# Alanlee0323/ISWM

Hardware: AMD Instinct MI355X
Metric: training images/sec (513x513) DeepLabV3+-ResNet101 (higher is better)
Workload: dtype f32; 1 GPU; deeplabv3plus_resnet101 output_stride=16, 513x513 synthetic tiles, 16 images/GPU (BASELINE.json configs[2]: global batch 128 over 8 GPUs), weighted CE [1,3], SGD-nesterov + cosine LR; fp32 tensors, conv products via six bf16 MFMAs on an exact 3-way operand split (bf16x6, fp32-level error); conv_math=bf16x6, global_batch=16, parallelism=dp1

## Files before the change

### include/iswm_hip.h

```cpp
#ifndef ISWM_HIP_H
#define ISWM_HIP_H

#include <stddef.h>
#include <stdint.h>

#ifdef __cplusplus
extern "C" {
#endif

typedef void* iswm_stream_t;

const char* iswm_last_error(void);
int iswm_version(void);

typedef struct {
    int N, H, W, Cin;
    int Ho, Wo, Cout;
    int KH, KW, stride, pad, dil;
    int ldx;
    int ldy;
} iswm_conv_desc;

int iswm_set_conv_math(int mode);
int iswm_get_conv_math(void);
int iswm_conv2d_kernel_name(const iswm_conv_desc* d, int kind, char* buf, int buflen);
int iswm_conv2d_stat_tile_rows(const iswm_conv_desc* d);
int iswm_conv2d_stat_tiles(const iswm_conv_desc* d);
int iswm_conv2d_fwd(const iswm_conv_desc* d, const float* x, const float* w, const float* bias,
                    float* y, float* stat_partials, iswm_stream_t stream);
int iswm_conv2d_dgrad(const iswm_conv_desc* d, const float* dy, const float* w, float* dx,
                      int accumulate, iswm_stream_t stream);
int iswm_transpose_weights(const iswm_conv_desc* d, const float* w, float* wt, iswm_stream_t stream);
int iswm_conv2d_dgrad_wants_wt(const iswm_conv_desc* d);
int iswm_conv2d_dgrad_wt(const iswm_conv_desc* d, const float* dy, const float* wt, float* dx, int accumulate,
                         iswm_stream_t stream);
size_t iswm_conv2d_packed_weight_bytes(const iswm_conv_desc* d, int kind);
int iswm_conv2d_pack_weights(const iswm_conv_desc* d, int kind, const float* w, void* packed, iswm_stream_t stream);
typedef struct iswm_pack_job {
    const float* w;
    void* packed;
    int Cout, taps, Cin, kind;
    int first_block, reserved;
} iswm_pack_job;
size_t iswm_packed_weight_bytes(int Cout, int taps, int Cin, int kind);
int iswm_pack_job_blocks(int Cout, int taps, int Cin, int kind);
int iswm_pack_weights_batch(const iswm_pack_job* jobs_dev, int njobs, int total_blocks, iswm_stream_t stream);
int iswm_conv2d_fwd_packed_stat_layout(const iswm_conv_desc* d, int* tiles, int* tile_rows);
int iswm_conv2d_fwd_packed(const iswm_conv_desc* d, const float* x, const void* wpk, const float* bias,
                           float* y, float* stat_partials, iswm_stream_t stream);
int iswm_conv2d_dgrad_packed(const iswm_conv_desc* d, const float* dy, const void* wpk, float* dx, int accumulate,
                             iswm_stream_t stream);
int iswm_split_planes(const float* x, int64_t M, int C, int ldx, void* planes, int ldp, int64_t plane_stride,
                      iswm_stream_t stream);
int iswm_join_planes(const void* planes, int ldp, int64_t plane_stride, int64_t M, int C, float* x, int ldx,
                     iswm_stream_t stream);
int iswm_bn_apply_pl(const float* y, int64_t M, int C, int ldy, const float* scale, const float* shift, const float* mean,
                     const void* residual, int ldr, int64_t res_ps, int relu, void* out, int ldo, int64_t out_ps,
                     iswm_stream_t stream);
int iswm_bn_backward_pl(const float* dout, int ldd, const void* out, int ldo, int64_t out_ps, const float* y, int ldy,
                        int64_t M, int C, const float* mean, const float* invstd, const float* gamma,
                        const float* mask_scale, const float* mask_shift, int relu, int training, float* dgamma,
                        float* dbeta, void* dy, int lddy, int64_t dy_ps, float* dres, int lddres, void* workspace,
                        size_t workspace_bytes, iswm_stream_t stream);
int iswm_maxpool3x3s2_fwd_pl(const float* x, int N, int H, int W, int C, void* y, int64_t y_ps, uint8_t* idx, int Ho,
                             int Wo, iswm_stream_t stream);
int iswm_gap_fwd_pl(const void* x, int64_t x_ps, int N, int HW, int C, int ldx, float* y, iswm_stream_t stream);
int iswm_bcast_fwd_pl(const float* v, int N, int HW, int C, void* y, int ldy, int64_t y_ps, iswm_stream_t stream);
int iswm_bilinear_fwd_pl(const float* x, int N, int Hi, int Wi, int C, int ldx, void* y, int64_t y_ps, int Ho, int Wo,
                         int ldy, iswm_stream_t stream);
size_t iswm_conv2d_pl2_weight_bytes(const iswm_conv_desc* d, int kind);
int iswm_conv2d_pl2_pack_weights(const iswm_conv_desc* d, int kind, const float* w, void* packed, iswm_stream_t stream);
int iswm_conv2d_pl2_tile_rows(const iswm_conv_desc* d, int kind);
int iswm_conv2d_fwd_pl2(const iswm_conv_desc* d, const void* xp, int64_t plane_stride, const void* wpk,
                        const float* bias, float* y, float* stat_partials, iswm_stream_t stream);
int iswm_conv2d_dgrad_pl2(const iswm_conv_desc* d, const void* dyp, int64_t plane_stride, const void* wpk,
                          float* dx, int accumulate, iswm_stream_t stream);
int iswm_conv2d_dgrad_pl2_stat_tiles(const iswm_conv_desc* d);
int iswm_conv2d_dgrad_pl2_bn(const iswm_conv_desc* d, const void* dyp, int64_t plane_stride, const void* wpk, float* dx,
                             int accumulate, const float* y, int ldy, const float* mean, const float* invstd,
                             const float* mask_scale, const float* mask_shift, int relu, const void* mask_hi,
                             int ld_mask, double* partials, int tiles, iswm_stream_t stream);
int iswm_bn_backward_stats_pl(const float* dout, int ldd, const void* out, int ldo, int64_t out_ps, const float* y, int ldy,
                              int64_t M, int C, const float* mean, const float* invstd, const float* gamma,
                              const float* mask_scale, const float* mask_shift, int relu, int training, float* dgamma,
                              float* dbeta, void* dy, int lddy, int64_t dy_ps, float* dres, int lddres,
                              const double* partials, int tiles, void* workspace, size_t workspace_bytes,
                              iswm_stream_t stream);
size_t iswm_aspp_plan_bytes(const iswm_conv_desc* d, int nbranch, const int* ksize, const int* dil, int kind);
int iswm_aspp_plan(const iswm_conv_desc* d, int nbranch, const int* ksize, const int* dil, int kind, void* host_plan,
                   int grid_hint);
int iswm_aspp_fwd(const iswm_conv_desc* d, int nbranch, const int* ksize, const int* dil, const void* plan_dev, const void* xp,
                  int64_t x_ps, const void* const* wpk, float* const* y, float* const* stats, iswm_stream_t stream);
int iswm_aspp_bwd(const iswm_conv_desc* d, int nbranch, const int* ksize, const int* dil, const void* plan_dev, const void* dyp,
                  int64_t dy_ps, int ld_dy, const void* const* wpk, float* dx, int accumulate, const void* xp, int64_t x_ps,
                  float* const* dw, float* workspace, size_t workspace_bytes, iswm_stream_t stream);
int iswm_conv2d_wgrad_planes_ok(const iswm_conv_desc* d);
size_t iswm_conv2d_wgrad_planes_workspace(const iswm_conv_desc* d);
int iswm_conv2d_wgrad_planes(const iswm_conv_desc* d, const void* xp, int64_t x_ps, const void* dyp, int64_t dy_ps, float* dw,
                             float* workspace, size_t workspace_bytes, iswm_stream_t stream);
int iswm_dwconv2d_fwd(const iswm_conv_desc* d, const float* x, const float* w, int Cw, const float* bias, float* y,
                      iswm_stream_t stream);
int iswm_dwconv2d_dgrad(const iswm_conv_desc* d, const float* dy, const float* w, int Cw, float* dx, int accumulate,
                        iswm_stream_t stream);
size_t iswm_dwconv2d_wgrad_workspace(const iswm_conv_desc* d);
int iswm_dwconv2d_wgrad(const iswm_conv_desc* d, const float* x, const float* dy, int Cw, float* dw, void* workspace,
                        size_t workspace_bytes, iswm_stream_t stream);
int iswm_dwconv3x3_stat_tile_rows(const iswm_conv_desc* d);
int iswm_dwconv3x3_stat_tiles(const iswm_conv_desc* d);
int iswm_dwconv3x3_fwd_stats(const iswm_conv_desc* d, const float* x, const float* w, int Cw, float* y,
                             float* stat_partials, iswm_stream_t stream);
size_t iswm_dwconv3x3_bwd_workspace(const iswm_conv_desc* d);
int iswm_dwconv3x3_bwd(const iswm_conv_desc* d, const float* x, const float* dy, const float* w, int Cw, float* dx,
                       int lddx, int accumulate, float* dw, void* workspace, size_t workspace_bytes, iswm_stream_t stream);
size_t iswm_conv2d_wgrad_workspace(const iswm_conv_desc* d);
int iswm_conv2d_wgrad(const iswm_conv_desc* d, const float* x, const float* dy, float* dw,
                      float* workspace, size_t workspace_bytes, iswm_stream_t stream);

int iswm_colstat_tiles(int64_t M);
int64_t iswm_colstat_tile_rows(int64_t M);
int iswm_colstat(const float* x, int64_t M, int C, int ld, float* partials, iswm_stream_t stream);
int iswm_bn_finalize(const float* partials, int tiles, int C, int64_t count, int64_t tile_rows,
                     const float* gamma, const float* beta, float* running_mean, float* running_var, float momentum,
                     float eps, float* scale, float* shift, float* save_mean, float* save_invstd,
                     iswm_stream_t stream);
int iswm_colstat_res(const float* x, int64_t M, int C, int ld, float* partials, iswm_stream_t stream);
int iswm_bn_finalize_res(const float* partials, int tiles, int C, int64_t count, int64_t tile_rows,
                         const float* gamma, const float* beta, float* running_mean, float* running_var, float momentum,
                         float eps, float* scale, float* shift, float* save_mean, float* save_invstd,
                         iswm_stream_t stream);
int iswm_bn_eval_coeffs(int C, const float* gamma, const float* beta, const float* running_mean,
                        const float* running_var, float eps, float* scale, float* shift,
                        float* save_mean, float* save_invstd, iswm_stream_t stream);
int iswm_bn_apply(const float* y, int64_t M, int C, int ldy, const float* scale, const float* shift,
                  const float* mean, const float* residual, int ldr, int relu, float* out, int ldo,
                  iswm_stream_t stream);
size_t iswm_bn_bwd_workspace(int64_t M, int C);
int iswm_bn_backward(const float* dout, int ldd, const float* out, int ldo, const float* y, int ldy,
                     int64_t M, int C, const float* mean, const float* invstd, const float* gamma,
                     const float* mask_scale, const float* mask_shift,
                     int relu, int training, float* dgamma, float* dbeta, float* dy, int lddy,
                     float* dres, int lddres, void* workspace, size_t workspace_bytes,
                     iswm_stream_t stream);
int iswm_colsum_finalize(const float* partials, int tiles, int C, float* out, float* scratch,
                         iswm_stream_t stream);

int iswm_maxpool3x3s2_fwd(const float* x, int N, int H, int W, int C, float* y, uint8_t* idx, int Ho,
                          int Wo, iswm_stream_t stream);
int iswm_maxpool3x3s2_bwd(const float* dy, const uint8_t* idx, int N, int H, int W, int C, int Ho,
                          int Wo, float* dx, iswm_stream_t stream);
int iswm_gap_fwd(const float* x, int N, int HW, int C, int ldx, float* y, iswm_stream_t stream);
int iswm_gap_bwd(const float* dy, int N, int HW, int C, float* dx, int lddx, int accumulate,
                 iswm_stream_t stream);
int iswm_bcast_fwd(const float* v, int N, int HW, int C, float* y, int ldy, iswm_stream_t stream);
int iswm_bcast_bwd(const float* dy, int lddy, int N, int HW, int C, float* dv, iswm_stream_t stream);

int iswm_bilinear_fwd(const float* x, int N, int Hi, int Wi, int C, int ldx, float* y, int Ho, int Wo,
                      int ldy, iswm_stream_t stream);
int iswm_bilinear_bwd(const float* dy, int N, int Hi, int Wi, int C, int lddy, int Ho, int Wo, float* dx,
                      int lddx, iswm_stream_t stream);
int iswm_bilinear_nhwc_to_nchw_fwd(const float* x, int N, int Hi, int Wi, int C, int ldx, float* y,
                                   int Ho, int Wo, iswm_stream_t stream);
int iswm_bilinear_nhwc_to_nchw_bwd(const float* dy, int N, int Hi, int Wi, int C, int lddx, int Ho,
                                   int Wo, float* dx, iswm_stream_t stream);

int iswm_nchw_to_nhwc(const float* x, int N, int C, int HW, float* y, int Cp, iswm_stream_t stream);
int iswm_nhwc_to_nchw(const float* x, int N, int C, int HW, int ldx, float* y, iswm_stream_t stream);
int iswm_copy_channels(const float* src, int lds, float* dst, int ldd, int64_t M, int C,
                       iswm_stream_t stream);
int iswm_add_inplace(float* dst, const float* src, int64_t n, iswm_stream_t stream);
int iswm_scale_inplace(float* x, int64_t n, const float* scalar_dev, float host_mul, iswm_stream_t stream);
int iswm_bn_apply_classify(const float* y, int64_t M, int C, int ldy, const float* scale, const float* shift, const float* mean,
                           const float* wc4, const float* bias4, float* logits, int ldl, iswm_stream_t stream);
size_t iswm_bn_classify_bwd_workspace(int64_t M, int C);
int iswm_bn_backward_classify(const float* dlogit, int ldl, const float* wc4, const float* y, int ldy, int64_t M, int C,
                              const float* mean, const float* invstd, const float* gamma, const float* mask_scale,
                              const float* mask_shift, int training, float* dgamma, float* dbeta, float* dwc4, void* dy, int lddy,
                              int64_t dy_ps, void* workspace, size_t workspace_bytes, iswm_stream_t stream);
int iswm_pad_weights(const float* w, int cout, int cin, int kh, int kw, const int64_t* strides, int cout_p, int cin_p, float* out_ohwi,
                     iswm_stream_t stream);
int iswm_unpad_weights(const float* dw_ohwi, int cout_p, int cin_p, int cout, int cin, int kh, int kw, float* grad,
                       const int64_t* strides, iswm_stream_t stream);
int iswm_fill_zero(void* p, size_t bytes, iswm_stream_t stream);
int iswm_zero_cols(void* y, int64_t M, int64_t ld_bytes, int byte0, int byte1, int64_t plane_bytes, int nplanes, iswm_stream_t stream);
int iswm_dropout_fwd(const float* x, float* y, uint8_t* mask, int64_t n, float p, uint64_t seed,
                     uint64_t offset, iswm_stream_t stream);
int iswm_dropout_bwd(const float* dy, const uint8_t* mask, float* dx, int64_t n, float p,
                     iswm_stream_t stream);

int iswm_loss_blocks(int64_t npix);
int iswm_loss_fwd(const float* logits, const void* labels, int label_bytes, int B, int C, int64_t HW,
                  const float* class_weight, int ignore_index, float alpha, float gamma, int mode,
                  float* grad_unnorm, float* partials, iswm_stream_t stream);
int iswm_loss_finalize(const float* partials, int blocks, int mode, int64_t npix, float* sums,
                       float* loss, iswm_stream_t stream);
int iswm_loss_bwd_scale(float* grad, int64_t n, const float* sums, const float* upstream, int mode,
                        int64_t npix, iswm_stream_t stream);
int iswm_overlap_loss_fwd(const float* logits, const void* labels, int label_bytes, int B, int C, int64_t HW,
                          const float* class_weight, int ignore_index, float* partials, double* sums,
                          iswm_stream_t stream);
int iswm_overlap_loss_coeffs(const double* sums, int C, double ce_weight, double overlap_weight, double alpha,
                             double beta, double gamma, double smooth, int classes, float* loss, float* coef,
                             iswm_stream_t stream);
int iswm_overlap_loss_bwd(const float* logits, const void* labels, int label_bytes, int B, int C, int64_t HW,
                          const float* class_weight, int ignore_index, const float* coef, const float* upstream,
                          float* grad, iswm_stream_t stream);
int iswm_argmax_nchw(const float* logits, int B, int C, int64_t HW, int64_t* out, iswm_stream_t stream);

int iswm_confusion_matrix(const void* labels, int label_dtype, const void* preds, int pred_dtype, int64_t npix,
                          int n_classes, int64_t* hist, iswm_stream_t stream);
int iswm_confusion_matrix_logits(const void* labels, int label_dtype, const float* logits, int B, int C, int64_t HW,
                                 int n_classes, int64_t* hist, iswm_stream_t stream);

int iswm_mask_morph(const void* src, int src_dtype, int N, int H, int W, int radius, int dilate, uint8_t* dst,
                    iswm_stream_t stream);
int iswm_ccl(const uint8_t* mask, int N, int H, int W, int32_t* labels, int32_t* areas, iswm_stream_t stream);
size_t iswm_mask_preprocess_workspace(int N, int H, int W);
int iswm_mask_preprocess(const void* src, int src_dtype, int N, int H, int W, uint8_t* out, double* weight,
                         int64_t* area, void* workspace, size_t workspace_bytes, iswm_stream_t stream);
int iswm_mask_fronts(const uint8_t* mask, const double* weight, int N, int H, int W, int32_t* fronts, int64_t* stats,
// ... 148 lines not shown
```

### iswm_amd/_lib.py

```python
import ctypes
import os
from ctypes import POINTER, Structure, c_char_p, c_double, c_float, c_int, c_int64, c_size_t, c_uint64, c_void_p

HERE = os.path.dirname(os.path.abspath(__file__))
LIB_PATH = os.path.join(HERE, "libiswm_hip.so")


class ConvDesc(Structure):
    _fields_ = [(n, c_int) for n in ("N", "H", "W", "Cin", "Ho", "Wo", "Cout", "KH", "KW", "stride", "pad",
                                     "dil", "ldx", "ldy")]


class QConvDesc(Structure):
    _fields_ = [(n, c_int) for n in ("N", "H", "W", "Cin", "Ho", "Wo", "Cout", "KH", "KW", "stride", "pad",
                                     "dil", "ldx", "ldy", "ldr", "relu", "lo", "out_f32", "cstore")]


class ScenePlan(Structure):
    _fields_ = [(n, c_int) for n in ("H", "W", "th", "tw", "sy", "sx", "nty", "ntx", "ramp")]

    @property
    def ntiles(self):
        return self.nty * self.ntx

    def origins_y(self):
        return [min(k * self.sy, self.H - self.th) for k in range(self.nty)]

    def origins_x(self):
        return [min(k * self.sx, self.W - self.tw) for k in range(self.ntx)]

    def astuple(self):
        return tuple(getattr(self, n) for n, _ in self._fields_)


class PredictView(Structure):
    _fields_ = [("yl", c_void_p), ("Hi", c_int), ("Wi", c_int), ("flip", c_int)]


P = c_void_p
_SIGS = {
    "iswm_last_error": (c_char_p, []),
    "iswm_version": (c_int, []),
    "iswm_set_conv_math": (c_int, [c_int]),
    "iswm_get_conv_math": (c_int, []),
    "iswm_conv2d_kernel_name": (c_int, [POINTER(ConvDesc), c_int, c_char_p, c_int]),
    "iswm_conv2d_stat_tile_rows": (c_int, [POINTER(ConvDesc)]),
    "iswm_conv2d_stat_tiles": (c_int, [POINTER(ConvDesc)]),
    "iswm_conv2d_fwd": (c_int, [POINTER(ConvDesc), P, P, P, P, P, P]),
    "iswm_conv2d_dgrad": (c_int, [POINTER(ConvDesc), P, P, P, c_int, P]),
    "iswm_transpose_weights": (c_int, [POINTER(ConvDesc), P, P, P]),
    "iswm_conv2d_dgrad_wants_wt": (c_int, [POINTER(ConvDesc)]),
    "iswm_conv2d_dgrad_wt": (c_int, [POINTER(ConvDesc), P, P, P, c_int, P]),
    "iswm_conv2d_packed_weight_bytes": (c_size_t, [POINTER(ConvDesc), c_int]),
    "iswm_conv2d_pack_weights": (c_int, [POINTER(ConvDesc), c_int, P, P, P]),
    "iswm_packed_weight_bytes": (c_size_t, [c_int, c_int, c_int, c_int]),
    "iswm_pack_job_blocks": (c_int, [c_int, c_int, c_int, c_int]),
    "iswm_pack_weights_batch": (c_int, [P, c_int, c_int, P]),
    "iswm_conv2d_fwd_packed_stat_layout": (c_int, [POINTER(ConvDesc), POINTER(c_int), POINTER(c_int)]),
    "iswm_conv2d_fwd_packed": (c_int, [POINTER(ConvDesc), P, P, P, P, P, P]),
    "iswm_conv2d_dgrad_packed": (c_int, [POINTER(ConvDesc), P, P, P, c_int, P]),
    "iswm_split_planes": (c_int, [P, c_int64, c_int, c_int, P, c_int, c_int64, P]),
    "iswm_join_planes": (c_int, [P, c_int, c_int64, c_int64, c_int, P, c_int, P]),
    "iswm_bn_apply_pl": (c_int, [P, c_int64, c_int, c_int, P, P, P, P, c_int, c_int64, c_int, P, c_int, c_int64, P]),
    "iswm_bn_backward_pl": (c_int, [P, c_int, P, c_int, c_int64, P, c_int, c_int64, c_int, P, P, P, P, P, c_int, c_int, P, P, P,
                                    c_int, c_int64, P, c_int, P, c_size_t, P]),
    "iswm_maxpool3x3s2_fwd_pl": (c_int, [P, c_int, c_int, c_int, c_int, P, c_int64, P, c_int, c_int, P]),
    "iswm_gap_fwd_pl": (c_int, [P, c_int64, c_int, c_int, c_int, c_int, P, P]),
    "iswm_bcast_fwd_pl": (c_int, [P, c_int, c_int, c_int, P, c_int, c_int64, P]),
    "iswm_bilinear_fwd_pl": (c_int, [P, c_int, c_int, c_int, c_int, c_int, P, c_int64, c_int, c_int, c_int, P]),
    "iswm_conv2d_pl2_weight_bytes": (c_size_t, [POINTER(ConvDesc), c_int]),
    "iswm_conv2d_pl2_pack_weights": (c_int, [POINTER(ConvDesc), c_int, P, P, P]),
    "iswm_conv2d_pl2_tile_rows": (c_int, [POINTER(ConvDesc), c_int]),
    "iswm_conv2d_fwd_pl2": (c_int, [POINTER(ConvDesc), P, c_int64, P, P, P, P, P]),
    "iswm_conv2d_dgrad_pl2": (c_int, [POINTER(ConvDesc), P, c_int64, P, P, c_int, P]),
    "iswm_conv2d_dgrad_pl2_stat_tiles": (c_int, [POINTER(ConvDesc)]),
    "iswm_conv2d_dgrad_pl2_bn": (c_int, [POINTER(ConvDesc), P, c_int64, P, P, c_int, P, c_int, P, P, P, P, c_int, P, c_int, P,
                                         c_int, P]),
    "iswm_bn_backward_stats_pl": (c_int, [P, c_int, P, c_int, c_int64, P, c_int, c_int64, c_int, P, P, P, P, P, c_int, c_int, P, P,
                                          P, c_int, c_int64, P, c_int, P, c_int, P, c_size_t, P]),
    "iswm_aspp_plan_bytes": (c_size_t, [POINTER(ConvDesc), c_int, POINTER(c_int), POINTER(c_int), c_int]),
    "iswm_aspp_plan": (c_int, [POINTER(ConvDesc), c_int, POINTER(c_int), POINTER(c_int), c_int, P, c_int]),
    "iswm_aspp_fwd": (c_int, [POINTER(ConvDesc), c_int, POINTER(c_int), POINTER(c_int), P, P, c_int64, POINTER(c_void_p),
                              POINTER(c_void_p), POINTER(c_void_p), P]),
    "iswm_aspp_bwd": (c_int, [POINTER(ConvDesc), c_int, POINTER(c_int), POINTER(c_int), P, P, c_int64, c_int, POINTER(c_void_p), P,
                              c_int, P, c_int64, POINTER(c_void_p), P, c_size_t, P]),
    "iswm_conv2d_wgrad_planes_ok": (c_int, [POINTER(ConvDesc)]),
    "iswm_conv2d_wgrad_planes_workspace": (c_size_t, [POINTER(ConvDesc)]),
    "iswm_conv2d_wgrad_planes": (c_int, [POINTER(ConvDesc), P, c_int64, P, c_int64, P, P, c_size_t, P]),
    "iswm_conv2d_wgrad_workspace": (c_size_t, [POINTER(ConvDesc)]),
    "iswm_dwconv2d_fwd": (c_int, [POINTER(ConvDesc), P, P, c_int, P, P, P]),
    "iswm_dwconv2d_dgrad": (c_int, [POINTER(ConvDesc), P, P, c_int, P, c_int, P]),
    "iswm_dwconv2d_wgrad_workspace": (c_size_t, [POINTER(ConvDesc)]),
    "iswm_dwconv2d_wgrad": (c_int, [POINTER(ConvDesc), P, P, c_int, P, P, c_size_t, P]),
    "iswm_dwconv3x3_stat_tile_rows": (c_int, [POINTER(ConvDesc)]),
    "iswm_dwconv3x3_stat_tiles": (c_int, [POINTER(ConvDesc)]),
    "iswm_dwconv3x3_fwd_stats": (c_int, [POINTER(ConvDesc), P, P, c_int, P, P, P]),
    "iswm_dwconv3x3_bwd_workspace": (c_size_t, [POINTER(ConvDesc)]),
    "iswm_dwconv3x3_bwd": (c_int, [POINTER(ConvDesc), P, P, P, c_int, P, c_int, c_int, P, P, c_size_t, P]),
    "iswm_conv2d_wgrad": (c_int, [POINTER(ConvDesc), P, P, P, P, c_size_t, P]),
    "iswm_colstat_tiles": (c_int, [c_int64]),
    "iswm_colstat_tile_rows": (c_int64, [c_int64]),
    "iswm_colstat": (c_int, [P, c_int64, c_int, c_int, P, P]),
    "iswm_bn_finalize": (c_int, [P, c_int, c_int, c_int64, c_int64, P, P, P, P, c_float, c_float, P, P, P, P, P]),
    "iswm_colstat_res": (c_int, [P, c_int64, c_int, c_int, P, P]),
    "iswm_bn_finalize_res": (c_int, [P, c_int, c_int, c_int64, c_int64, P, P, P, P, c_float, c_float, P, P, P, P, P]),
    "iswm_bn_eval_coeffs": (c_int, [c_int, P, P, P, P, c_float, P, P, P, P, P]),
    "iswm_bn_apply": (c_int, [P, c_int64, c_int, c_int, P, P, P, P, c_int, c_int, P, c_int, P]),
    "iswm_bn_bwd_workspace": (c_size_t, [c_int64, c_int]),
    "iswm_bn_backward": (c_int, [P, c_int, P, c_int, P, c_int, c_int64, c_int, P, P, P, P, P, c_int, c_int, P, P, P, c_int,
                                 P, c_int, P, c_size_t, P]),
    "iswm_colsum_finalize": (c_int, [P, c_int, c_int, P, P, P]),
    "iswm_maxpool3x3s2_fwd": (c_int, [P, c_int, c_int, c_int, c_int, P, P, c_int, c_int, P]),
    "iswm_maxpool3x3s2_bwd": (c_int, [P, P, c_int, c_int, c_int, c_int, c_int, c_int, P, P]),
    "iswm_gap_fwd": (c_int, [P, c_int, c_int, c_int, c_int, P, P]),
    "iswm_gap_bwd": (c_int, [P, c_int, c_int, c_int, P, c_int, c_int, P]),
    "iswm_bcast_fwd": (c_int, [P, c_int, c_int, c_int, P, c_int, P]),
    "iswm_bcast_bwd": (c_int, [P, c_int, c_int, c_int, c_int, P, P]),
    "iswm_bilinear_fwd": (c_int, [P, c_int, c_int, c_int, c_int, c_int, P, c_int, c_int, c_int, P]),
    "iswm_bilinear_bwd": (c_int, [P, c_int, c_int, c_int, c_int, c_int, c_int, c_int, P, c_int, P]),
    "iswm_bilinear_nhwc_to_nchw_fwd": (c_int, [P, c_int, c_int, c_int, c_int, c_int, P, c_int, c_int, P]),
    "iswm_bilinear_nhwc_to_nchw_bwd": (c_int, [P, c_int, c_int, c_int, c_int, c_int, c_int, c_int, P, P]),
    "iswm_nchw_to_nhwc": (c_int, [P, c_int, c_int, c_int, P, c_int, P]),
    "iswm_nhwc_to_nchw": (c_int, [P, c_int, c_int, c_int, c_int, P, P]),
    "iswm_copy_channels": (c_int, [P, c_int, P, c_int, c_int64, c_int, P]),
    "iswm_add_inplace": (c_int, [P, P, c_int64, P]),
    "iswm_scale_inplace": (c_int, [P, c_int64, P, c_float, P]),
    "iswm_bn_apply_classify": (c_int, [P, c_int64, c_int, c_int, P, P, P, P, P, P, c_int, P]),
    "iswm_bn_classify_bwd_workspace": (c_size_t, [c_int64, c_int]),
    "iswm_bn_backward_classify": (c_int, [P, c_int, P, P, c_int, c_int64, c_int, P, P, P, P, P, c_int, P, P, P, P, c_int, c_int64,
                                          P, c_size_t, P]),
    "iswm_pad_weights": (c_int, [P, c_int, c_int, c_int, c_int, P, c_int, c_int, P, P]),
    "iswm_unpad_weights": (c_int, [P, c_int, c_int, c_int, c_int, c_int, c_int, P, P, P]),
    "iswm_fill_zero": (c_int, [P, c_size_t, P]),
    "iswm_zero_cols": (c_int, [P, c_int64, c_int64, c_int, c_int, c_int64, c_int, P]),
    "iswm_dropout_fwd": (c_int, [P, P, P, c_int64, c_float, c_uint64, c_uint64, P]),
    "iswm_dropout_bwd": (c_int, [P, P, P, c_int64, c_float, P]),
    "iswm_loss_blocks": (c_int, [c_int64]),
    "iswm_loss_fwd": (c_int, [P, P, c_int, c_int, c_int, c_int64, P, c_int, c_float, c_float, c_int, P, P, P]),
    "iswm_loss_finalize": (c_int, [P, c_int, c_int, c_int64, P, P, P]),
    "iswm_loss_bwd_scale": (c_int, [P, c_int64, P, P, c_int, c_int64, P]),
    "iswm_overlap_loss_fwd": (c_int, [P, P, c_int, c_int, c_int, c_int64, P, c_int, P, P, P]),
    "iswm_overlap_loss_coeffs": (c_int, [P, c_int, c_double, c_double, c_double, c_double, c_double, c_double, c_int, P, P, P]),
    "iswm_overlap_loss_bwd": (c_int, [P, P, c_int, c_int, c_int, c_int64, P, c_int, P, P, P, P]),
    "iswm_argmax_nchw": (c_int, [P, c_int, c_int, c_int64, P, P]),
    "iswm_augment_batch": (c_int, [P, P, P, P, c_int, c_int, c_int, POINTER(c_float), POINTER(c_float), P, P, P]),
    "iswm_aug_rotate": (c_int, [P, P, P, P, c_int, c_int64, P, c_size_t, P, c_size_t, P]),
    "iswm_augment_batch_ex_workspace": (c_size_t, [c_int, c_int, c_int]),
    "iswm_augment_batch_ex": (c_int, [P, P, P, P, P, P, P, c_int, c_int, c_int, POINTER(c_float), POINTER(c_float), c_int, P,
                                      P, P, c_size_t, P]),
    "iswm_label_prepare_workspace": (c_size_t, [c_int64]),
    "iswm_label_prepare": (c_int, [P, c_int64, P, P, c_size_t, P]),
    "iswm_label_count_workspace": (c_size_t, [c_int64]),
    "iswm_label_count": (c_int, [P, c_int64, c_int, P, P, c_size_t, P]),
    "iswm_aug_tables_workspace": (c_size_t, [P, c_int]),
    "iswm_aug_tables": (c_int, [P, c_int, c_int, P, c_size_t, P]),
    "iswm_gather_normalize": (c_int, [P, P, P, c_int, c_int, c_int, POINTER(c_float), POINTER(c_float), P, P, P]),
    "iswm_confusion_matrix": (c_int, [P, c_int, P, c_int, c_int64, c_int, P, P]),
    "iswm_confusion_matrix_logits": (c_int, [P, c_int, P, c_int, c_int, c_int64, c_int, P, P]),
    "iswm_mask_morph": (c_int, [P, c_int, c_int, c_int, c_int, c_int, c_int, P, P]),
    "iswm_ccl": (c_int, [P, c_int, c_int, c_int, P, P, P]),
    "iswm_mask_preprocess_workspace": (c_size_t, [c_int, c_int, c_int]),
    "iswm_mask_preprocess": (c_int, [P, c_int, c_int, c_int, c_int, P, P, P, P, c_size_t, P]),
    "iswm_mask_fronts": (c_int, [P, P, c_int, c_int, c_int, P, P, P]),
    "iswm_front_error": (c_int, [P, P, c_int, c_int, c_double, P, P]),
    "iswm_mask_pair_scores": (c_int, [P, P, P, P, P, c_int, c_int, c_int, P, P, P]),
    "iswm_region_workspace": (c_size_t, [c_int, c_int, c_int]),
    "iswm_region_score": (c_int, [P, c_int, P, c_int, c_int, c_int, c_int, P, P, P, c_size_t, P]),
    "iswm_predict_normalize": (c_int, [P, c_int, c_int, c_int, POINTER(c_float), POINTER(c_float), P, P]),
    "iswm_predict_maps_workspace": (c_size_t, [c_int, c_int, c_int]),
    "iswm_predict_maps": (c_int, [P, c_int, c_int, c_int, c_int, c_int, c_int, c_int, c_int, c_float, c_int, c_int, P, P,
                                  P, P, P, P, c_size_t, P]),
    "iswm_scene_plan_make": (c_int, [c_int, c_int, c_int, c_int, POINTER(ScenePlan)]),
    "iswm_scene_tiles_normalize": (c_int, [P, POINTER(ScenePlan), c_int, c_int, POINTER(c_float), POINTER(c_float), P, P]),
    "iswm_scene_maps_workspace": (c_size_t, [c_int, c_int]),
    "iswm_scene_maps": (c_int, [P, POINTER(ScenePlan), c_int, c_int, c_int, c_int, c_int, c_float, c_int, c_int, P, P, P, P,
                                P, P, c_size_t, P]),
    "iswm_predict_view_normalize": (c_int, [P, c_int, c_int, c_int, c_int, c_int, c_int, POINTER(c_float), POINTER(c_float),
                                            P, P]),
    "iswm_predict_views_maps_workspace": (c_size_t, [c_int, c_int, c_int]),
    "iswm_predict_views_maps": (c_int, [POINTER(PredictView), c_int, c_int, c_int, c_int, c_int, c_int, c_int, c_float,
                                        c_int, c_int, P, P, P, P, P, P, c_size_t, P]),
    "iswm_val_panels": (c_int, [P, P, P, c_int, c_int, c_int, c_int, c_int, c_int, c_int, c_int, POINTER(c_float),
                                POINTER(c_float), P, P, P, P, P, P, P, P, P, P]),
    "iswm_qconv_weight_bytes": (c_size_t, [POINTER(QConvDesc)]),
    "iswm_qconv_fwd": (c_int, [POINTER(QConvDesc), P, P, P, P, P, c_double, c_double, P, P]),
    "iswm_absmax_workspace": (c_size_t, [c_int64, c_int]),
    "iswm_absmax": (c_int, [P, c_int64, c_int64, c_int, c_int, P, c_size_t, P, P]),
    "iswm_quantize_i8": (c_int, [P, c_int64, c_int64, c_int, c_int, c_double, c_int, P, c_int, P]),
    "iswm_qgap": (c_int, [P, c_int, c_int, c_int, c_int, c_double, c_double, P, c_int, P]),
    "iswm_qbcast": (c_int, [P, c_int, c_int, c_int, c_int, P, c_int, P]),
    "iswm_qbilinear": (c_int, [P, c_int, c_int, c_int, c_int, c_int, c_double, c_int, c_int, c_double, P, c_int, P]),
    "iswm_sgd_step": (c_int, [P, P, P, c_int64, P, c_float, c_float, c_int, P]),
    "iswm_adam_step": (c_int, [P, P, P, P, c_int64, P, c_float, c_float, c_float, c_float, c_int, P]),
    "iswm_grad_sqnorm_slots": (c_int, []),
    "iswm_grad_sqnorm": (c_int, [P, c_int64, P, c_int, P]),
    "iswm_clip_finalize": (c_int, [P, c_float, P, P]),
    "iswm_sgd_step_ex": (c_int, [P, P, P, c_int64, P, c_float, c_float, c_int, P, P, P]),
    "iswm_adam_step_ex": (c_int, [P, P, P, P, c_int64, P, c_float, c_float, c_float, c_float, c_int, P, P, P]),
    "iswm_swap_f32": (c_int, [P, P, c_int64, P]),
}

EXPORTS = tuple(_SIGS)
_lib = None


class IswmError(RuntimeError):
    pass


def load():
    global _lib
    if _lib is not None:
        return _lib
    if not os.path.exists(LIB_PATH):
        raise ImportError(
            "libiswm_hip.so is not built (%s). Run `python -m iswm_amd.build` (hipcc, gfx950). "
            "iswm_amd has no CPU or torch-op fallback." % LIB_PATH)
    import torch
    lib = ctypes.CDLL(LIB_PATH)
    for name, (res, args) in _SIGS.items():
# ... 14 lines not shown
```

### iswm_amd/csrc/bn.hip

```cpp
#include <stdlib.h>

#include "rowmap.h"

namespace iswm {

template <bool RES>
__global__ __launch_bounds__(256) void k_colstat(const float* __restrict__ x, int64_t M, int C4, int ld,
                                                 int CQ, int RL, int tiles, int C, int64_t R,
                                                 float* __restrict__ partials) {
    __shared__ float red[256 * 4];
    __shared__ float mean_s[256 * 4];
    RowThread rt = row_thread(C4, CQ, RL);
    const int t = threadIdx.x;
    const int64_t r_begin = (int64_t)blockIdx.x * R;
    const int64_t r_end = min(M, r_begin + R);
    const float cnt = (float)(r_end - r_begin);
    const float* p = x + rt.c4 * 4;
    float4 s = make_float4(0, 0, 0, 0);
    if (rt.active)
        for (int64_t r = r_begin + rt.rl; r < r_end; r += RL) {
            float4 v = ld4(p + r * ld);
            s.x += v.x; s.y += v.y; s.z += v.z; s.w += v.w;
        }
    st4(&red[t * 4], s);
    __syncthreads();
    if (rt.active && rt.rl == 0) {
        for (int k = 1; k < RL; ++k) {
            float4 a = ld4(&red[(t + k * CQ) * 4]);
            s.x += a.x; s.y += a.y; s.z += a.z; s.w += a.w;
        }
        st4(&partials[(size_t)blockIdx.x * C + rt.c4 * 4], s);
        st4(&mean_s[t * 4], make_float4(s.x / cnt, s.y / cnt, s.z / cnt, s.w / cnt));
    }
    __syncthreads();
    float4 q = make_float4(0, 0, 0, 0), rs = q;
    if (rt.active) {
        const float4 mu = ld4(&mean_s[(t - rt.rl * CQ) * 4]);
        for (int64_t r = r_begin + rt.rl; r < r_end; r += RL) {
            float4 v = ld4(p + r * ld);
            float dx = v.x - mu.x, dy = v.y - mu.y, dz = v.z - mu.z, dw = v.w - mu.w;
            q.x += dx * dx; q.y += dy * dy; q.z += dz * dz; q.w += dw * dw;
            if (RES) { rs.x += dx; rs.y += dy; rs.z += dz; rs.w += dw; }
        }
    }
    st4(&red[t * 4], q);
    __syncthreads();
    if (rt.active && rt.rl == 0) {
        for (int k = 1; k < RL; ++k) {
            float4 a = ld4(&red[(t + k * CQ) * 4]);
            q.x += a.x; q.y += a.y; q.z += a.z; q.w += a.w;
        }
        st4(&partials[(size_t)(tiles + blockIdx.x) * C + rt.c4 * 4], q);
    }
    if (RES) {
        __syncthreads();
        st4(&red[t * 4], rs);
        __syncthreads();
        if (rt.active && rt.rl == 0) {
            for (int k = 1; k < RL; ++k) {
                float4 a = ld4(&red[(t + k * CQ) * 4]);
                rs.x += a.x; rs.y += a.y; rs.z += a.z; rs.w += a.w;
            }
            st4(&partials[(size_t)(2 * tiles + blockIdx.x) * C + rt.c4 * 4], rs);
        }
    }
}

template <int CPB>
__global__ __launch_bounds__(256) void k_bn_finalize(const float* __restrict__ partials, int tiles, int C,
                                                     double count, double R, const float* __restrict__ gamma,
                                                     const float* __restrict__ beta, float* running_mean,
                                                     float* running_var, float momentum, float eps,
                                                     float* scale, float* shift, float* save_mean,
                                                     float* save_invstd) {
    constexpr int TL = 256 / CPB;
    __shared__ double red[TL][CPB + 1];
    __shared__ double mean_s[CPB];
    const int cl = threadIdx.x % CPB, tl = threadIdx.x / CPB;
    const int c = blockIdx.x * CPB + cl;
    constexpr int KEEP = 8;
    float sv[KEEP], qv[KEEP];
    double s = 0.0;
    if (c < C) {
#pragma unroll
        for (int i = 0; i < KEEP; ++i) {
            const int k = tl + i * TL;
            sv[i] = k < tiles ? partials[(size_t)k * C + c] : 0.f;
            qv[i] = k < tiles ? partials[(size_t)(tiles + k) * C + c] : 0.f;
        }
#pragma unroll
        for (int i = 0; i < KEEP; ++i) s += (double)sv[i];
        for (int k = tl + KEEP * TL; k < tiles; k += TL) s += (double)partials[(size_t)k * C + c];
    }
    red[tl][cl] = s;
    __syncthreads();
    if (tl == 0) {
        for (int k = 1; k < TL; ++k) s += red[k][cl];
        mean_s[cl] = s / count;
    }
    __syncthreads();
    const double mean = mean_s[cl];
    double m2 = 0.0;
    if (c < C) {
        auto term = [&](int k, float sk, float qk) -> double {
            const double nt = R > 0.0 ? fmin(R, count - (double)k * R) : (double)partials[(size_t)2 * tiles * C + k];
            const double d = (double)sk / nt - mean;
            return (double)qk + nt * d * d;
        };
#pragma unroll
        for (int i = 0; i < KEEP; ++i) {
            const int k = tl + i * TL;
            if (k < tiles) m2 += term(k, sv[i], qv[i]);
        }
        for (int k = tl + KEEP * TL; k < tiles; k += TL) m2 += term(k, partials[(size_t)k * C + c], partials[(size_t)(tiles + k) * C + c]);
    }
    __syncthreads();
    red[tl][cl] = m2;
    __syncthreads();
    if (tl == 0 && c < C) {
        for (int k = 1; k < TL; ++k) m2 += red[k][cl];
        double var = m2 / count;
        if (var < 0.0) var = 0.0;
        float invstd = (float)(1.0 / sqrt(var + (double)eps));
        float g = gamma ? gamma[c] : 1.f, b = beta ? beta[c] : 0.f;
        float sc = g * invstd;
        scale[c] = sc;
        shift[c] = b;
        save_mean[c] = (float)mean;
        save_invstd[c] = invstd;
        if (running_mean) {
            double unbiased = count > 1.0 ? var * count / (count - 1.0) : var;
            running_mean[c] = (1.f - momentum) * running_mean[c] + momentum * (float)mean;
            running_var[c] = (1.f - momentum) * running_var[c] + momentum * (float)unbiased;
        }
    }
}

__global__ __launch_bounds__(256) void k_bn_finalize_res(const float* __restrict__ partials, int tiles, int C, double count,
                                                         double R, const float* __restrict__ gamma,
                                                         const float* __restrict__ beta, float* running_mean,
                                                         float* running_var, float momentum, float eps, float* scale,
                                                         float* shift, float* save_mean, float* save_invstd) {
    constexpr int CPB = 4, TL = 64;
    __shared__ double red[TL][CPB + 1];
    __shared__ double mean_s[CPB];
    const int cl = threadIdx.x % CPB, tl = threadIdx.x / CPB;
    const int c = blockIdx.x * CPB + cl;
    auto rows = [&](int k) -> double { return fmin(R, count - (double)k * R); };
    auto centre = [&](int k) -> double { return (double)(partials[(size_t)k * C + c] / (float)rows(k)); };
    double s = 0.0;
    if (c < C)
        for (int k = tl; k < tiles; k += TL) s += rows(k) * centre(k) + (double)partials[(size_t)(2 * tiles + k) * C + c];
    red[tl][cl] = s;
    __syncthreads();
    if (tl == 0) {
        for (int k = 1; k < TL; ++k) s += red[k][cl];
        mean_s[cl] = s / count;
    }
    __syncthreads();
    const double mean = mean_s[cl];
    double m2 = 0.0;
    if (c < C)
        for (int k = tl; k < tiles; k += TL) {
            const double d = centre(k) - mean;
            m2 += (double)partials[(size_t)(tiles + k) * C + c] + 2.0 * d * (double)partials[(size_t)(2 * tiles + k) * C + c] +
                  rows(k) * d * d;
        }
    __syncthreads();
    red[tl][cl] = m2;
    __syncthreads();
    if (tl == 0 && c < C) {
        for (int k = 1; k < TL; ++k) m2 += red[k][cl];
        double var = m2 / count;
        if (var < 0.0) var = 0.0;
        const float invstd = (float)(1.0 / sqrt(var + (double)eps));
        const float g = gamma ? gamma[c] : 1.f, b = beta ? beta[c] : 0.f;
        scale[c] = g * invstd;
        shift[c] = b;
        save_mean[c] = (float)mean;
        save_invstd[c] = invstd;
        if (running_mean) {
            const double unbiased = count > 1.0 ? var * count / (count - 1.0) : var;
            running_mean[c] = (1.f - momentum) * running_mean[c] + momentum * (float)mean;
            running_var[c] = (1.f - momentum) * running_var[c] + momentum * (float)unbiased;
        }
    }
}

__global__ void k_bn_eval_coeffs(int C, const float* gamma, const float* beta, const float* rm,
                                 const float* rv, float eps, float* scale, float* shift, float* save_mean,
                                 float* save_invstd) {
    int c = blockIdx.x * blockDim.x + threadIdx.x;
    if (c >= C) return;
    float invstd = 1.f / sqrtf(rv[c] + eps);
    float g = gamma ? gamma[c] : 1.f, b = beta ? beta[c] : 0.f;
    float sc = g * invstd;
    scale[c] = sc;
    shift[c] = b;
    save_mean[c] = rm[c];
    save_invstd[c] = invstd;
}

template <int RELU, bool RES>
__global__ __launch_bounds__(256) void k_bn_apply(const float* __restrict__ y, int64_t M, int C4, int ldy,
                                                  const float* __restrict__ scale,
                                                  const float* __restrict__ shift,
                                                  const float* __restrict__ mean,
                                                  const void* __restrict__ res, int ldr, int64_t rps,
                                                  void* __restrict__ out, int ldo, int64_t ops, int CQ, int RL) {
    RowThread rt = row_thread(C4, CQ, RL);
    if (!rt.active) return;
    const int c = rt.c4 * 4;
    const float4 sc = ld4(scale + c), sh = ld4(shift + c), mu = ld4(mean + c);
    for (int64_t r = rt.row0; r < M; r += rt.rstep) {
        float4 v = ld4(y + r * ldy + c);
        float4 o;
        o.x = (v.x - mu.x) * sc.x + sh.x; o.y = (v.y - mu.y) * sc.y + sh.y;
        o.z = (v.z - mu.z) * sc.z + sh.z; o.w = (v.w - mu.w) * sc.w + sh.w;
        if (RES) {
            float4 q = ld4x(res, r * ldr + c, rps);
            o.x += q.x; o.y += q.y; o.z += q.z; o.w += q.w;
        }
        if (RELU) {
            o.x = fmaxf(o.x, 0.f); o.y = fmaxf(o.y, 0.f); o.z = fmaxf(o.z, 0.f); o.w = fmaxf(o.w, 0.f);
        }
        if (RELU == 2) {
            o.x = fminf(o.x, 6.f); o.y = fminf(o.y, 6.f); o.z = fminf(o.z, 6.f); o.w = fminf(o.w, 6.f);
        }
        st4x(out, r * ldo + c, ops, o);
    }
}

template <int RELU, bool RES>
__global__ __launch_bounds__(256) void k_bn_apply8(const float* __restrict__ y, int64_t M, int C8, int ldy,
                                                   const float* __restrict__ scale, const float* __restrict__ shift,
                                                   const float* __restrict__ mean, const void* __restrict__ res, int ldr,
                                                   int64_t rps, void* __restrict__ out, int ldo, int64_t ops, int CQ, int RL) {
    RowThread rt = row_thread(C8, CQ, RL);
    if (!rt.active) return;
    const int c = rt.c4 * 8;
    const float4 sc0 = ld4(scale + c), sc1 = ld4(scale + c + 4), sh0 = ld4(shift + c), sh1 = ld4(shift + c + 4);
    const float4 mu0 = ld4(mean + c), mu1 = ld4(mean + c + 4);
    auto one = [&](int64_t r, const float4 v0, const float4 v1, const float4 q0, const float4 q1) {
        float4 o0, o1;
        o0.x = (v0.x - mu0.x) * sc0.x + sh0.x; o0.y = (v0.y - mu0.y) * sc0.y + sh0.y;
        o0.z = (v0.z - mu0.z) * sc0.z + sh0.z; o0.w = (v0.w - mu0.w) * sc0.w + sh0.w;
        o1.x = (v1.x - mu1.x) * sc1.x + sh1.x; o1.y = (v1.y - mu1.y) * sc1.y + sh1.y;
        o1.z = (v1.z - mu1.z) * sc1.z + sh1.z; o1.w = (v1.w - mu1.w) * sc1.w + sh1.w;
        if (RES) {
            o0.x += q0.x; o0.y += q0.y; o0.z += q0.z; o0.w += q0.w;
            o1.x += q1.x; o1.y += q1.y; o1.z += q1.z; o1.w += q1.w;
        }
        if (RELU) {
            o0.x = fmaxf(o0.x, 0.f); o0.y = fmaxf(o0.y, 0.f); o0.z = fmaxf(o0.z, 0.f); o0.w = fmaxf(o0.w, 0.f);
            o1.x = fmaxf(o1.x, 0.f); o1.y = fmaxf(o1.y, 0.f); o1.z = fmaxf(o1.z, 0.f); o1.w = fmaxf(o1.w, 0.f);
        }
        if (RELU == 2) {
            o0.x = fminf(o0.x, 6.f); o0.y = fminf(o0.y, 6.f); o0.z = fminf(o0.z, 6.f); o0.w = fminf(o0.w, 6.f);
            o1.x = fminf(o1.x, 6.f); o1.y = fminf(o1.y, 6.f); o1.z = fminf(o1.z, 6.f); o1.w = fminf(o1.w, 6.f);
        }
        st8x(out, r * ldo + c, ops, o0, o1);
    };
    int64_t r = rt.row0;
    const float4 z4 = make_float4(0.f, 0.f, 0.f, 0.f);
    for (; r + rt.rstep < M; r += 2 * rt.rstep) {
        const int64_t r2 = r + rt.rstep;
        const float4 a0 = ld4(y + r * ldy + c), a1 = ld4(y + r * ldy + c + 4);
        const float4 b0 = ld4(y + r2 * ldy + c), b1 = ld4(y + r2 * ldy + c + 4);
        float4 qa0 = z4, qa1 = z4, qb0 = z4, qb1 = z4;
        if (RES) {
            ld8x(res, r * ldr + c, rps, qa0, qa1);
            ld8x(res, r2 * ldr + c, rps, qb0, qb1);
        }
        one(r, a0, a1, qa0, qa1);
        one(r2, b0, b1, qb0, qb1);
    }
    if (r < M) {
        const float4 a0 = ld4(y + r * ldy + c), a1 = ld4(y + r * ldy + c + 4);
        float4 qa0 = z4, qa1 = z4;
        if (RES) ld8x(res, r * ldr + c, rps, qa0, qa1);
        one(r, a0, a1, qa0, qa1);
    }
}

template <int RELU, bool DBL>
__global__ __launch_bounds__(256) void k_bn_bwd_reduce(const float* __restrict__ dout, int ldd,
                                                       const void* __restrict__ out, int ldo, int64_t ops,
                                                       const float* __restrict__ y, int ldy, int64_t M,
                                                       int C4, int C, const float* __restrict__ mean,
                                                       const float* __restrict__ invstd,
                                                       const float* __restrict__ mscale,
                                                       const float* __restrict__ mshift, int CQ, int RL,
                                                       int tiles, double* __restrict__ partials) {
    __shared__ double red[2 * 256 * 4];
    RowThread rt = row_thread(C4, CQ, RL);
    double s[4] = {0, 0, 0, 0}, s2[4] = {0, 0, 0, 0};
    if (rt.active) {
        const int c = rt.c4 * 4;
        const float4 mu = ld4(mean + c), is = ld4(invstd + c);
        float4 msc = make_float4(0.f, 0.f, 0.f, 0.f), msh = msc;
        if (RELU == 2) {
            msc = ld4(mscale + c);
            msh = ld4(mshift + c);
        }
        for (int64_t r = rt.row0; r < M; r += 8 * rt.rstep) {
            float f[4] = {0.f, 0.f, 0.f, 0.f}, f2[4] = {0.f, 0.f, 0.f, 0.f};
#pragma unroll
            for (int u = 0; u < 8; ++u) {
                const int64_t rr = r + u * rt.rstep;
                if (rr < M) {
                    float4 g = ld4(dout + rr * ldd + c);
                    float4 v = ld4(y + rr * ldy + c);
                    if (RELU == 1) {
                        float4 o = ld4x_hi(out, rr * ldo + c, ops);
                        g.x = o.x > 0.f ? g.x : 0.f; g.y = o.y > 0.f ? g.y : 0.f;
                        g.z = o.z > 0.f ? g.z : 0.f; g.w = o.w > 0.f ? g.w : 0.f;
                    } else if (RELU == 3) {
                        float4 o = ld4x_hi(out, rr * ldo + c, ops);
                        g.x = (o.x > 0.f && o.x < 6.f) ? g.x : 0.f; g.y = (o.y > 0.f && o.y < 6.f) ? g.y : 0.f;
                        g.z = (o.z > 0.f && o.z < 6.f) ? g.z : 0.f; g.w = (o.w > 0.f && o.w < 6.f) ? g.w : 0.f;
                    } else if (RELU == 2) {
                        g.x = (v.x - mu.x) * msc.x + msh.x > 0.f ? g.x : 0.f;
                        g.y = (v.y - mu.y) * msc.y + msh.y > 0.f ? g.y : 0.f;
                        g.z = (v.z - mu.z) * msc.z + msh.z > 0.f ? g.z : 0.f;
                        g.w = (v.w - mu.w) * msc.w + msh.w > 0.f ? g.w : 0.f;
                    }
                    if (DBL) {
                        const double gd[4] = {g.x, g.y, g.z, g.w}, vd[4] = {v.x, v.y, v.z, v.w};
                        const double mud[4] = {mu.x, mu.y, mu.z, mu.w}, isd[4] = {is.x, is.y, is.z, is.w};
#pragma unroll
                        for (int k = 0; k < 4; ++k) {
                            s[k] += gd[k];
                            s2[k] += gd[k] * ((vd[k] - mud[k]) * isd[k]);
                        }
                    } else {
                        f[0] += g.x; f[1] += g.y; f[2] += g.z; f[3] += g.w;
                        f2[0] += g.x * ((v.x - mu.x) * is.x); f2[1] += g.y * ((v.y - mu.y) * is.y);
                        f2[2] += g.z * ((v.z - mu.z) * is.z); f2[3] += g.w * ((v.w - mu.w) * is.w);
                    }
                }
            }
#pragma unroll
            for (int k = 0; k < 4; ++k) {
                s[k] += (double)f[k];
                s2[k] += (double)f2[k];
            }
        }
    }
    const int t = threadIdx.x;
#pragma unroll
    for (int k = 0; k < 4; ++k) {
        red[t * 4 + k] = s[k];
        red[(256 + t) * 4 + k] = s2[k];
    }
    __syncthreads();
    if (rt.active && rt.rl == 0) {
        for (int j = 1; j < RL; ++j)
#pragma unroll
            for (int k = 0; k < 4; ++k) {
                s[k] += red[(t + j * CQ) * 4 + k];
                s2[k] += red[(256 + t + j * CQ) * 4 + k];
            }
#pragma unroll
        for (int k = 0; k < 4; ++k) {
            partials[(size_t)blockIdx.x * C + rt.c4 * 4 + k] = s[k];
            partials[(size_t)(tiles + blockIdx.x) * C + rt.c4 * 4 + k] = s2[k];
        }
    }
}

template <typename T, int CPB>
__global__ __launch_bounds__(256) void k_bn_bwd_finalize(const T* __restrict__ partials, int tiles, int C,
                                                         float* dgamma, float* dbeta, double* sums) {
    constexpr int TL = 256 / CPB;
    __shared__ double red[2][TL][CPB + 1];
    const int cl = threadIdx.x % CPB, tl = threadIdx.x / CPB;
    const int c = blockIdx.x * CPB + cl;
    double s = 0.0, s2 = 0.0;
    if (c < C) {
        int k = tl;
        for (; k + TL < tiles; k += 2 * TL) {
            const T a0 = partials[(size_t)k * C + c], a1 = partials[(size_t)(k + TL) * C + c];
            const T b0 = partials[(size_t)(tiles + k) * C + c], b1 = partials[(size_t)(tiles + k + TL) * C + c];
            s += (double)a0 + (double)a1;
            s2 += (double)b0 + (double)b1;
        }
        for (; k < tiles; k += TL) {
            s += (double)partials[(size_t)k * C + c];
            s2 += (double)partials[(size_t)(tiles + k) * C + c];
        }
    }
    red[0][tl][cl] = s;
    red[1][tl][cl] = s2;
    __syncthreads();
    if (tl == 0 && c < C) {
        for (int k = 1; k < TL; ++k) {
            s += red[0][k][cl];
            s2 += red[1][k][cl];
        }
        dbeta[c] = (float)s;
        dgamma[c] = (float)s2;
        if (sums) {
            sums[c] = s;
            sums[C + c] = s2;
        }
    }
}

template <int RELU, bool TRAIN, bool DRES>
__global__ __launch_bounds__(256) void k_bn_bwd_apply(const float* __restrict__ dout, int ldd,
                                                      const void* __restrict__ out, int ldo, int64_t ops,
                                                      const float* __restrict__ y, int ldy, int64_t M,
                                                      int C4, int C, const float* __restrict__ mean,
                                                      const float* __restrict__ invstd,
                                                      const float* __restrict__ gamma,
                                                      const float* __restrict__ mscale,
                                                      const float* __restrict__ mshift,
                                                      const double* __restrict__ sums, double inv_count,
                                                      void* __restrict__ dy, int lddy, int64_t dyps,
                                                      float* __restrict__ dres, int lddres, int CQ, int RL) {
    RowThread rt = row_thread(C4, CQ, RL);
    if (!rt.active) return;
    const int c = rt.c4 * 4;
    const float4 mu = ld4(mean + c), is = ld4(invstd + c);
    const float4 ga = gamma ? ld4(gamma + c) : make_float4(1.f, 1.f, 1.f, 1.f);
    const double mud[4] = {mu.x, mu.y, mu.z, mu.w}, isd[4] = {is.x, is.y, is.z, is.w};
    const double gi[4] = {(double)ga.x * is.x, (double)ga.y * is.y, (double)ga.z * is.z, (double)ga.w * is.w};
    float4 msc = make_float4(0.f, 0.f, 0.f, 0.f), msh = msc;
    if (RELU == 2) {
        msc = ld4(mscale + c);
        msh = ld4(mshift + c);
    }
    double k1[4] = {0, 0, 0, 0}, k2[4] = {0, 0, 0, 0};
    if (TRAIN) {
#pragma unroll
        for (int k = 0; k < 4; ++k) {
            k1[k] = sums[c + k] * inv_count;
            k2[k] = sums[C + c + k] * inv_count;
        }
    }
    for (int64_t r = rt.row0; r < M; r += rt.rstep) {
        float4 g = ld4(dout + r * ldd + c);
        float4 v = make_float4(0.f, 0.f, 0.f, 0.f);
        if (TRAIN || RELU == 2) v = ld4(y + r * ldy + c);
        if (RELU == 1) {
            float4 o = ld4x_hi(out, r * ldo + c, ops);
            g.x = o.x > 0.f ? g.x : 0.f; g.y = o.y > 0.f ? g.y : 0.f;
            g.z = o.z > 0.f ? g.z : 0.f; g.w = o.w > 0.f ? g.w : 0.f;
        } else if (RELU == 3) {
            float4 o = ld4x_hi(out, r * ldo + c, ops);
            g.x = (o.x > 0.f && o.x < 6.f) ? g.x : 0.f; g.y = (o.y > 0.f && o.y < 6.f) ? g.y : 0.f;
            g.z = (o.z > 0.f && o.z < 6.f) ? g.z : 0.f; g.w = (o.w > 0.f && o.w < 6.f) ? g.w : 0.f;
        } else if (RELU == 2) {
            g.x = (v.x - mu.x) * msc.x + msh.x > 0.f ? g.x : 0.f;
            g.y = (v.y - mu.y) * msc.y + msh.y > 0.f ? g.y : 0.f;
            g.z = (v.z - mu.z) * msc.z + msh.z > 0.f ? g.z : 0.f;
            g.w = (v.w - mu.w) * msc.w + msh.w > 0.f ? g.w : 0.f;
        }
        if (DRES) st4(dres + r * lddres + c, g);
        const double gd[4] = {g.x, g.y, g.z, g.w};
        float d[4];
        if (TRAIN) {
            const double vd[4] = {v.x, v.y, v.z, v.w};
#pragma unroll
            for (int k = 0; k < 4; ++k)
                d[k] = (float)(gi[k] * (gd[k] - k1[k] - (vd[k] - mud[k]) * isd[k] * k2[k]));
        } else {
#pragma unroll
            for (int k = 0; k < 4; ++k) d[k] = (float)(gi[k] * gd[k]);
        }
        st4x(dy, r * lddy + c, dyps, make_float4(d[0], d[1], d[2], d[3]));
    }
}

static int chk_rows(const char* what, int64_t M, int C, int ld) {
    ISWM_REQUIRE(M > 0 && C > 0 && C % 4 == 0 && ld % 4 == 0 && ld >= C, "%s: bad shape M=%lld C=%d ld=%d", what,
                 (long long)M, C, ld);
    return 0;
}

}

using namespace iswm;

extern "C" int iswm_colstat_tiles(int64_t M) {
    int64_t t = (M + 31) / 32;
    if (t > 1024) t = 1024;
    if (t < 1) t = 1;
    return (int)t;
}

extern "C" int64_t iswm_colstat_tile_rows(int64_t M) {
    const int64_t tiles = iswm_colstat_tiles(M);
    return (M + tiles - 1) / tiles;
}

extern "C" int iswm_colstat(const float* x, int64_t M, int C, int ld, float* partials, iswm_stream_t stream) {
    if (int e = chk_rows("colstat", M, C, ld)) return e;
    ISWM_REQUIRE(x && partials && aligned16(x) && aligned16(partials), "colstat: bad pointer");
    const int64_t R = iswm_colstat_tile_rows(M);
    const int tiles = (int)((M + R - 1) / R);
    RowPlan p = plan_rows(M, C, tiles);
    hipLaunchKernelGGL((k_colstat<false>), dim3(p.rowblocks, p.colblocks), dim3(256), 0, (hipStream_t)stream, x, M, p.C4,
                       ld, p.CQ, p.RL, tiles, C, R, partials);
    return check_launch("colstat");
}

extern "C" int iswm_colstat_res(const float* x, int64_t M, int C, int ld, float* partials, iswm_stream_t stream) {
    if (int e = chk_rows("colstat_res", M, C, ld)) return e;
    ISWM_REQUIRE(x && partials && aligned16(x) && aligned16(partials), "colstat_res: bad pointer");
    const int64_t R = iswm_colstat_tile_rows(M);
    const int tiles = (int)((M + R - 1) / R);
    RowPlan p = plan_rows(M, C, tiles);
    hipLaunchKernelGGL((k_colstat<true>), dim3(p.rowblocks, p.colblocks), dim3(256), 0, (hipStream_t)stream, x, M, p.C4,
                       ld, p.CQ, p.RL, tiles, C, R, partials);
    return check_launch("colstat_res");
}

extern "C" int iswm_bn_finalize(const float* partials, int tiles, int C, int64_t count, int64_t tile_rows,
                                const float* gamma, const float* beta, float* running_mean, float* running_var, float momentum,
                                float eps, float* scale, float* shift, float* save_mean, float* save_invstd,
                                iswm_stream_t stream) {
    ISWM_REQUIRE(partials && scale && shift && save_mean && save_invstd && tiles > 0 && C > 0 && count > 0 &&
                     tile_rows >= 0 && (tile_rows == 0 || (int64_t)tiles == (count + tile_rows - 1) / tile_rows),
                 "bn_finalize: bad argument (tiles %d, count %lld, tile_rows %lld)", tiles, (long long)count,
                 (long long)tile_rows);
    if (tiles > 512)
        hipLaunchKernelGGL((k_bn_finalize<1>), dim3(C), dim3(256), 0, (hipStream_t)stream, partials, tiles, C,
                           (double)count, (double)tile_rows, gamma, beta, running_mean, running_var, momentum, eps,
                           scale, shift, save_mean, save_invstd);
    else if (tiles > 32)
        hipLaunchKernelGGL((k_bn_finalize<4>), dim3((C + 3) / 4), dim3(256), 0, (hipStream_t)stream, partials, tiles, C,
                           (double)count, (double)tile_rows, gamma, beta, running_mean, running_var, momentum, eps,
                           scale, shift, save_mean, save_invstd);
    else
        hipLaunchKernelGGL((k_bn_finalize<16>), dim3((C + 15) / 16), dim3(256), 0, (hipStream_t)stream, partials, tiles,
                           C, (double)count, (double)tile_rows, gamma, beta, running_mean, running_var, momentum, eps,
                           scale, shift, save_mean, save_invstd);
    return check_launch("bn_finalize");
}

extern "C" int iswm_bn_finalize_res(const float* partials, int tiles, int C, int64_t count, int64_t tile_rows,
                                    const float* gamma, const float* beta, float* running_mean, float* running_var,
                                    float momentum, float eps, float* scale, float* shift, float* save_mean,
                                    float* save_invstd, iswm_stream_t stream) {
    ISWM_REQUIRE(partials && scale && shift && save_mean && save_invstd && tiles > 0 && C > 0 && count > 0 && tile_rows > 0 &&
                     (int64_t)tiles == (count + tile_rows - 1) / tile_rows,
                 "bn_finalize_res: bad argument (tiles %d, count %lld, tile_rows %lld)", tiles, (long long)count,
                 (long long)tile_rows);
    hipLaunchKernelGGL(k_bn_finalize_res, dim3((C + 3) / 4), dim3(256), 0, (hipStream_t)stream, partials, tiles, C,
                       (double)count, (double)tile_rows, gamma, beta, running_mean, running_var, momentum, eps, scale, shift,
                       save_mean, save_invstd);
    return check_launch("bn_finalize_res");
}

extern "C" int iswm_bn_eval_coeffs(int C, const float* gamma, const float* beta, const float* running_mean,
                                   const float* running_var, float eps, float* scale, float* shift,
                                   float* save_mean, float* save_invstd, iswm_stream_t stream) {
    ISWM_REQUIRE(C > 0 && running_mean && running_var && scale && shift && save_mean && save_invstd,
                 "bn_eval_coeffs: bad argument");
    hipLaunchKernelGGL(k_bn_eval_coeffs, dim3((C + 255) / 256), dim3(256), 0, (hipStream_t)stream, C, gamma, beta,
                       running_mean, running_var, eps, scale, shift, save_mean, save_invstd);
    return check_launch("bn_eval_coeffs");
}

static int chk_ps(const char* what, const void* p, int64_t M, int ld, int64_t ps) {
    ISWM_REQUIRE(ps == 0 || ps == -1 || (ps >= M * ld && ps % 4 == 0), "%s: bad plane stride %lld", what, (long long)ps);
    ISWM_REQUIRE(ps == 0 ? aligned16(p) : ((reinterpret_cast<uintptr_t>(p) & 7) == 0), "%s: misaligned tensor", what);
    return 0;
}

extern "C" int iswm_bn_apply(const float* y, int64_t M, int C, int ldy, const float* scale, const float* shift,
                             const float* mean, const float* residual, int ldr, int relu, float* out, int ldo,
                             iswm_stream_t stream) {
    return iswm_bn_apply_pl(y, M, C, ldy, scale, shift, mean, residual, ldr, 0, relu, out, ldo, 0, stream);
}

extern "C" int iswm_bn_apply_pl(const float* y, int64_t M, int C, int ldy, const float* scale, const float* shift,
                                const float* mean, const void* residual, int ldr, int64_t res_ps, int relu, void* out,
                                int ldo, int64_t out_ps, iswm_stream_t stream) {
    if (int e = chk_rows("bn_apply", M, C, ldy)) return e;
    ISWM_REQUIRE(y && scale && shift && mean && out && ldo % 4 == 0 && ldo >= C, "bn_apply: bad argument");
    ISWM_REQUIRE(!residual || (ldr % 4 == 0 && ldr >= C), "bn_apply: bad residual pitch");
    if (int e = chk_ps("bn_apply(out)", out, M, ldo, out_ps)) return e;
    if (residual) if (int e = chk_ps("bn_apply(residual)", residual, M, ldr, res_ps)) return e;
    const int64_t rps = res_ps, ops = out_ps;
    hipStream_t s = (hipStream_t)stream;
    if (out_ps != 0 && C % 8 == 0 && ldy % 8 == 0 && ldo % 8 == 0 && aligned16(out) && (out_ps < 0 || out_ps % 8 == 0) &&
        (!residual || (ldr % 8 == 0 && aligned16(residual) && (res_ps <= 0 || res_ps % 8 == 0)))) {
        RowPlan p = plan_rows(M, C / 2);
        dim3 grid(p.rowblocks, p.colblocks), blk(256);
#define LAUNCH8(R, S) \
    hipLaunchKernelGGL((k_bn_apply8<R, S>), grid, blk, 0, s, y, M, p.C4, ldy, scale, shift, mean, residual, ldr, rps, out, \
                       ldo, ops, p.CQ, p.RL)
        ISWM_REQUIRE(relu == 0 || relu == 1 || relu == 6, "bn_apply: relu must be 0 (none), 1 (ReLU) or 6 (ReLU6)");
        if (relu == 6 && residual) LAUNCH8(2, true);
        else if (relu == 6) LAUNCH8(2, false);
        else if (relu && residual) LAUNCH8(1, true);
        else if (relu) LAUNCH8(1, false);
        else if (residual) LAUNCH8(0, true);
        else LAUNCH8(0, false);
#undef LAUNCH8
        return check_launch("bn_apply8");
    }
    RowPlan p = plan_rows(M, C);
    dim3 grid(p.rowblocks, p.colblocks), blk(256);
#define LAUNCH(R, S) \
    hipLaunchKernelGGL((k_bn_apply<R, S>), grid, blk, 0, s, y, M, p.C4, ldy, scale, shift, mean, residual, ldr, rps, out, \
                       ldo, ops, \
                       p.CQ, p.RL)
    ISWM_REQUIRE(relu == 0 || relu == 1 || relu == 6, "bn_apply: relu must be 0 (none), 1 (ReLU) or 6 (ReLU6)");
    if (relu == 6 && residual) LAUNCH(2, true);
    else if (relu == 6) LAUNCH(2, false);
    else if (relu && residual) LAUNCH(1, true);
    else if (relu) LAUNCH(1, false);
    else if (residual) LAUNCH(0, true);
    else LAUNCH(0, false);
#undef LAUNCH
    return check_launch("bn_apply");
}

extern "C" size_t iswm_bn_bwd_workspace(int64_t M, int C) {
    return ((size_t)2 * iswm_colstat_tiles(M) * C + (size_t)2 * C) * sizeof(double);
}

extern "C" int iswm_bn_backward(const float* dout, int ldd, const float* out, int ldo, const float* y, int ldy,
                                int64_t M, int C, const float* mean, const float* invstd, const float* gamma,
                                const float* mask_scale, const float* mask_shift,
                                int relu, int training, float* dgamma, float* dbeta, float* dy, int lddy,
                                float* dres, int lddres, void* workspace, size_t workspace_bytes,
                                iswm_stream_t stream) {
    return iswm_bn_backward_pl(dout, ldd, out, ldo, 0, y, ldy, M, C, mean, invstd, gamma, mask_scale, mask_shift, relu,
                               training, dgamma, dbeta, dy, lddy, 0, dres, lddres, workspace, workspace_bytes, stream);
}

static int bn_backward_impl(const float* dout, int ldd, const void* out, int ldo, int64_t out_ps, const float* y,
                            int ldy, int64_t M, int C, const float* mean, const float* invstd, const float* gamma,
                            const float* mask_scale, const float* mask_shift, int relu, int training,
                            float* dgamma, float* dbeta, void* dy, int lddy, int64_t dy_ps, float* dres,
                            int lddres, void* workspace, size_t workspace_bytes, const double* ready_partials,
                            int ready_tiles, iswm_stream_t stream) {
    if (int e = chk_rows("bn_backward", M, C, ldy)) return e;
    if (int e = chk_ps("bn_backward(dy)", dy, M, lddy, dy_ps)) return e;
    if (out) if (int e = chk_ps("bn_backward(out)", out, M, ldo, out_ps)) return e;
    const int64_t ops = out_ps, dyps = dy_ps;
    ISWM_REQUIRE(relu == 0 || relu == 1 || relu == 6, "bn_backward: relu must be 0 (none), 1 (ReLU) or 6 (ReLU6)");
    const bool relu6 = relu == 6;
    const bool masky = relu == 1 && !dres && mask_scale && mask_shift;
    ISWM_REQUIRE(dout && y && mean && invstd && dgamma && dbeta && dy && workspace && (!relu || out || masky),
                 "bn_backward: null pointer");
    ISWM_REQUIRE(ldd % 4 == 0 && ldd >= C && lddy % 4 == 0 && lddy >= C && (!relu || (ldo % 4 == 0 && ldo >= C)) &&
                     (!dres || (lddres % 4 == 0 && lddres >= C)),
                 "bn_backward: bad pitch");
    ISWM_REQUIRE(workspace_bytes >= iswm_bn_bwd_workspace(M, C) && aligned16(workspace),
                 "bn_backward: workspace too small");
    const int tiles = ready_partials ? ready_tiles : iswm_colstat_tiles(M);
    const double* partials = ready_partials ? ready_partials : (const double*)workspace;
    double* sums = (double*)workspace + (size_t)2 * iswm_colstat_tiles(M) * C;
    hipStream_t s = (hipStream_t)stream;
    if (!ready_partials) {
        double* partials = (double*)workspace;
        RowPlan p = plan_rows(M, C, tiles);
        dim3 grid(p.rowblocks, p.colblocks), blk(256);
#define RLAUNCH(R, D)                                                                                           \
    hipLaunchKernelGGL((k_bn_bwd_reduce<R, D>), grid, blk, 0, s, dout, ldd, out, ldo, ops, y, ldy, M, p.C4, C, mean, invstd, \
                       mask_scale, mask_shift, p.CQ, p.RL, tiles, partials)
        const bool dbl = M <= 8192;
        if (relu6 && dbl) RLAUNCH(3, true);
        else if (relu6) RLAUNCH(3, false);
        else if (masky && dbl) RLAUNCH(2, true);
        else if (masky) RLAUNCH(2, false);
        else if (relu && dbl) RLAUNCH(1, true);
        else if (relu) RLAUNCH(1, false);
        else if (dbl) RLAUNCH(0, true);
        else RLAUNCH(0, false);
#undef RLAUNCH
        if (int e = check_launch("bn_bwd_reduce")) return e;
    }
    if (tiles > 32)
        hipLaunchKernelGGL((k_bn_bwd_finalize<double, 4>), dim3((C + 3) / 4), dim3(256), 0, s, partials, tiles, C,
                           dgamma, dbeta, sums);
    else
        hipLaunchKernelGGL((k_bn_bwd_finalize<double, 16>), dim3((C + 15) / 16), dim3(256), 0, s, partials, tiles, C,
                           dgamma, dbeta, sums);
    if (int e = check_launch("bn_bwd_finalize")) return e;
    const double inv = 1.0 / (double)M;
    RowPlan p = plan_rows(M, C);
    dim3 grid(p.rowblocks, p.colblocks), blk(256);
#define LAUNCH(R, T, D)                                                                                          \
    hipLaunchKernelGGL((k_bn_bwd_apply<R, T, D>), grid, blk, 0, s, dout, ldd, out, ldo, ops, y, ldy, M, p.C4, C, mean,    \
                       invstd, gamma, mask_scale, mask_shift, sums, inv, dy, lddy, dyps, dres, lddres, p.CQ, p.RL)
    const int key = (relu ? 4 : 0) | (training ? 2 : 0) | (dres ? 1 : 0);
    if (relu6) {
        if (training && dres) LAUNCH(3, true, true);
        else if (training) LAUNCH(3, true, false);
        else if (dres) LAUNCH(3, false, true);
        else LAUNCH(3, false, false);
    } else if (masky) {
        if (training) LAUNCH(2, true, false);
        else LAUNCH(2, false, false);
    } else switch (key) {
        case 0: LAUNCH(0, false, false); break;
        case 1: LAUNCH(0, false, true); break;
        case 2: LAUNCH(0, true, false); break;
        case 3: LAUNCH(0, true, true); break;
        case 4: LAUNCH(1, false, false); break;
        case 5: LAUNCH(1, false, true); break;
        case 6: LAUNCH(1, true, false); break;
        default: LAUNCH(1, true, true); break;
    }
#undef LAUNCH
    return check_launch("bn_bwd_apply");
}

extern "C" int iswm_bn_backward_pl(const float* dout, int ldd, const void* out, int ldo, int64_t out_ps, const float* y,
                                   int ldy, int64_t M, int C, const float* mean, const float* invstd, const float* gamma,
                                   const float* mask_scale, const float* mask_shift, int relu, int training,
                                   float* dgamma, float* dbeta, void* dy, int lddy, int64_t dy_ps, float* dres,
                                   int lddres, void* workspace, size_t workspace_bytes, iswm_stream_t stream) {
    return bn_backward_impl(dout, ldd, out, ldo, out_ps, y, ldy, M, C, mean, invstd, gamma, mask_scale, mask_shift, relu,
                            training, dgamma, dbeta, dy, lddy, dy_ps, dres, lddres, workspace, workspace_bytes, nullptr, 0,
                            stream);
}

extern "C" int iswm_bn_backward_stats_pl(const float* dout, int ldd, const void* out, int ldo, int64_t out_ps,
                                         const float* y, int ldy, int64_t M, int C, const float* mean,
                                         const float* invstd, const float* gamma, const float* mask_scale,
                                         const float* mask_shift, int relu, int training, float* dgamma, float* dbeta,
                                         void* dy, int lddy, int64_t dy_ps, float* dres, int lddres,
                                         const double* partials, int tiles, void* workspace, size_t workspace_bytes,
                                         iswm_stream_t stream) {
    ISWM_REQUIRE(partials && tiles > 0 && aligned16(partials), "bn_backward_stats: bad partials");
    return bn_backward_impl(dout, ldd, out, ldo, out_ps, y, ldy, M, C, mean, invstd, gamma, mask_scale, mask_shift, relu,
                            training, dgamma, dbeta, dy, lddy, dy_ps, dres, lddres, workspace, workspace_bytes, partials,
                            tiles, stream);
}

extern "C" int iswm_colsum_finalize(const float* partials, int tiles, int C, float* out, float* scratch,
                                    iswm_stream_t stream) {
    ISWM_REQUIRE(partials && out && scratch && tiles > 0 && C > 0, "colsum_finalize: bad argument");
    hipLaunchKernelGGL((k_bn_bwd_finalize<float, 4>), dim3((C + 3) / 4), dim3(256), 0, (hipStream_t)stream, partials,
                       tiles, C, scratch, out, (double*)nullptr);
    return check_launch("colsum_finalize");
}
```

### iswm_amd/csrc/pool.hip

```cpp
#include "rowmap.h"

namespace iswm {

__global__ __launch_bounds__(256) void k_maxpool_fwd(const float* __restrict__ x, int N, int H, int W, int C4,
                                                     void* __restrict__ y, int64_t yps, uint8_t* __restrict__ idx, int Ho,
                                                     int Wo, int CQ, int RL) {
    RowThread rt = row_thread(C4, CQ, RL);
    if (!rt.active) return;
    const int C = C4 * 4, c = rt.c4 * 4;
    const int64_t Mo = (int64_t)N * Ho * Wo;
    for (int64_t r = rt.row0; r < Mo; r += rt.rstep) {
        int n = (int)(r / (Ho * Wo));
        int rem = (int)(r - (int64_t)n * Ho * Wo);
        int oh = rem / Wo, ow = rem - oh * Wo;
        const int hs = oh * 2 - 1, ws = ow * 2 - 1;
        float4 best = make_float4(-INFINITY, -INFINITY, -INFINITY, -INFINITY);
        int bi[4] = {-1, -1, -1, -1};
#pragma unroll
        for (int kh = 0; kh < 3; ++kh) {
            int ih = hs + kh;
            if (ih < 0 || ih >= H) continue;
#pragma unroll
            for (int kw = 0; kw < 3; ++kw) {
                int iw = ws + kw;
                if (iw < 0 || iw >= W) continue;
                float4 v = ld4(x + ((size_t)(n * H + ih) * W + iw) * C + c);
                const int tap = kh * 3 + kw;
                if (bi[0] < 0 || v.x > best.x || v.x != v.x) { best.x = v.x; bi[0] = tap; }
                if (bi[1] < 0 || v.y > best.y || v.y != v.y) { best.y = v.y; bi[1] = tap; }
                if (bi[2] < 0 || v.z > best.z || v.z != v.z) { best.z = v.z; bi[2] = tap; }
                if (bi[3] < 0 || v.w > best.w || v.w != v.w) { best.w = v.w; bi[3] = tap; }
            }
        }
        st4x(y, (int64_t)r * C + c, yps, best);
        uchar4 u = make_uchar4((unsigned char)bi[0], (unsigned char)bi[1], (unsigned char)bi[2],
                               (unsigned char)bi[3]);
        *reinterpret_cast<uchar4*>(idx + (size_t)r * C + c) = u;
    }
}

__global__ __launch_bounds__(256) void k_maxpool_bwd(const float* __restrict__ dy,
                                                     const uint8_t* __restrict__ idx, int N, int H, int W,
                                                     int C4, int Ho, int Wo, float* __restrict__ dx, int CQ,
                                                     int RL) {
    RowThread rt = row_thread(C4, CQ, RL);
    if (!rt.active) return;
    const int C = C4 * 4, c = rt.c4 * 4;
    const int64_t Mi = (int64_t)N * H * W;
    for (int64_t r = rt.row0; r < Mi; r += rt.rstep) {
        int n = (int)(r / (H * W));
        int rem = (int)(r - (int64_t)n * H * W);
        int ih = rem / W, iw = rem - ih * W;
        float4 g = make_float4(0, 0, 0, 0);
        const int oh_lo = ih >> 1, oh_hi = (ih + 1) >> 1;
        const int ow_lo = iw >> 1, ow_hi = (iw + 1) >> 1;
        for (int oh = oh_lo; oh <= oh_hi; ++oh) {
            if (oh >= Ho) continue;
            const int kh = ih - (oh * 2 - 1);
            for (int ow = ow_lo; ow <= ow_hi; ++ow) {
                if (ow >= Wo) continue;
                const int kw = iw - (ow * 2 - 1);
                const unsigned char tap = (unsigned char)(kh * 3 + kw);
                size_t o = ((size_t)(n * Ho + oh) * Wo + ow) * C + c;
                uchar4 u = *reinterpret_cast<const uchar4*>(idx + o);
                float4 d = ld4(dy + o);
                if (u.x == tap) g.x += d.x;
                if (u.y == tap) g.y += d.y;
                if (u.z == tap) g.z += d.z;
                if (u.w == tap) g.w += d.w;
            }
        }
        st4(dx + (size_t)r * C + c, g);
    }
}

__global__ __launch_bounds__(256) void k_gap_fwd(const void* __restrict__ x, int64_t xps, int HW, int C4, int ldx,
                                                 float* __restrict__ y, int CQ, int RL) {
    __shared__ float red[256 * 4];
    RowThread rt = row_thread(C4, CQ, RL);
    const int n = blockIdx.z;
    float4 s = make_float4(0, 0, 0, 0);
    if (rt.active) {
        const int64_t p = (int64_t)n * HW * ldx + rt.c4 * 4;
        float4 s1 = s, s2 = s, s3 = s;
        int r = rt.rl;
        for (; r + 3 * RL < HW; r += 4 * RL) {
            const float4 v0 = ld4x(x, p + (int64_t)r * ldx, xps), v1 = ld4x(x, p + (int64_t)(r + RL) * ldx, xps);
            const float4 v2 = ld4x(x, p + (int64_t)(r + 2 * RL) * ldx, xps), v3 = ld4x(x, p + (int64_t)(r + 3 * RL) * ldx, xps);
            s.x += v0.x; s.y += v0.y; s.z += v0.z; s.w += v0.w;
            s1.x += v1.x; s1.y += v1.y; s1.z += v1.z; s1.w += v1.w;
            s2.x += v2.x; s2.y += v2.y; s2.z += v2.z; s2.w += v2.w;
            s3.x += v3.x; s3.y += v3.y; s3.z += v3.z; s3.w += v3.w;
        }
        for (; r < HW; r += RL) {
            const float4 v = ld4x(x, p + (int64_t)r * ldx, xps);
            s.x += v.x; s.y += v.y; s.z += v.z; s.w += v.w;
        }
        s.x = (s.x + s1.x) + (s2.x + s3.x); s.y = (s.y + s1.y) + (s2.y + s3.y);
        s.z = (s.z + s1.z) + (s2.z + s3.z); s.w = (s.w + s1.w) + (s2.w + s3.w);
    }
    const int t = threadIdx.x;
    st4(&red[t * 4], s);
    __syncthreads();
    if (rt.active && rt.rl == 0) {
        for (int k = 1; k < RL; ++k) {
            float4 a = ld4(&red[(t + k * CQ) * 4]);
            s.x += a.x; s.y += a.y; s.z += a.z; s.w += a.w;
        }
        const float inv = 1.f / (float)HW;
        st4(y + (size_t)n * C4 * 4 + rt.c4 * 4, make_float4(s.x * inv, s.y * inv, s.z * inv, s.w * inv));
    }
}

template <bool ACC>
__global__ __launch_bounds__(256) void k_bcast(const float* __restrict__ v, int HW, int C4, float mul,
                                               void* __restrict__ dst, int ldd, int64_t dps, int CQ, int RL) {
    RowThread rt = row_thread(C4, CQ, RL);
    if (!rt.active) return;
    const int n = blockIdx.z, c = rt.c4 * 4;
    float4 s = ld4(v + (size_t)n * C4 * 4 + c);
    s = make_float4(s.x * mul, s.y * mul, s.z * mul, s.w * mul);
    const int64_t p = (int64_t)n * HW * ldd + c;
    for (int64_t r = rt.row0; r < HW; r += rt.rstep) {
        if (ACC) {
            float* q = reinterpret_cast<float*>(dst) + p + r * ldd;
            float4 o = ld4(q);
            st4(q, make_float4(o.x + s.x, o.y + s.y, o.z + s.z, o.w + s.w));
        } else {
            st4x(dst, p + r * ldd, dps, s);
        }
    }
}

__global__ __launch_bounds__(256) void k_bcast_bwd(const float* __restrict__ dy, int HW, int C4, int ldd,
                                                   float* __restrict__ dv, int CQ, int RL) {
    __shared__ float red[256 * 4];
    RowThread rt = row_thread(C4, CQ, RL);
    const int n = blockIdx.z;
    float4 s = make_float4(0, 0, 0, 0);
    if (rt.active) {
        const float* p = dy + (size_t)n * HW * ldd + rt.c4 * 4;
        float4 s1 = s, s2 = s, s3 = s;
        int r = rt.rl;
        for (; r + 3 * RL < HW; r += 4 * RL) {
            const float4 v0 = ld4(p + (size_t)r * ldd), v1 = ld4(p + (size_t)(r + RL) * ldd);
            const float4 v2 = ld4(p + (size_t)(r + 2 * RL) * ldd), v3 = ld4(p + (size_t)(r + 3 * RL) * ldd);
            s.x += v0.x; s.y += v0.y; s.z += v0.z; s.w += v0.w;
            s1.x += v1.x; s1.y += v1.y; s1.z += v1.z; s1.w += v1.w;
            s2.x += v2.x; s2.y += v2.y; s2.z += v2.z; s2.w += v2.w;
            s3.x += v3.x; s3.y += v3.y; s3.z += v3.z; s3.w += v3.w;
        }
        for (; r < HW; r += RL) {
            const float4 v = ld4(p + (size_t)r * ldd);
            s.x += v.x; s.y += v.y; s.z += v.z; s.w += v.w;
        }
        s.x = (s.x + s1.x) + (s2.x + s3.x); s.y = (s.y + s1.y) + (s2.y + s3.y);
        s.z = (s.z + s1.z) + (s2.z + s3.z); s.w = (s.w + s1.w) + (s2.w + s3.w);
    }
    const int t = threadIdx.x;
    st4(&red[t * 4], s);
    __syncthreads();
    if (rt.active && rt.rl == 0) {
        for (int k = 1; k < RL; ++k) {
            float4 a = ld4(&red[(t + k * CQ) * 4]);
            s.x += a.x; s.y += a.y; s.z += a.z; s.w += a.w;
        }
        st4(dv + (size_t)n * C4 * 4 + rt.c4 * 4, s);
    }
}

static RowPlan plan_reduce(int C) {
    RowPlan p;
    p.C4 = C / 4;
    p.CQ = p.C4 < 32 ? p.C4 : 32;
    p.RL = 256 / p.CQ;
    p.colblocks = (p.C4 + p.CQ - 1) / p.CQ;
    p.rowblocks = 1;
    return p;
}

}

using namespace iswm;

extern "C" int iswm_maxpool3x3s2_fwd(const float* x, int N, int H, int W, int C, float* y, uint8_t* idx, int Ho,
                                     int Wo, iswm_stream_t stream) {
    return iswm_maxpool3x3s2_fwd_pl(x, N, H, W, C, y, 0, idx, Ho, Wo, stream);
}

extern "C" int iswm_maxpool3x3s2_fwd_pl(const float* x, int N, int H, int W, int C, void* y, int64_t y_ps, uint8_t* idx,
                                        int Ho, int Wo, iswm_stream_t stream) {
    ISWM_REQUIRE(x && y && idx && C % 4 == 0 && N > 0, "maxpool_fwd: bad argument");
    ISWM_REQUIRE(y_ps == 0 || y_ps == -1 || y_ps >= (int64_t)N * Ho * Wo * C, "maxpool_fwd: bad plane stride");
    const int64_t yps = y_ps;
    ISWM_REQUIRE(Ho == (H + 2 - 3) / 2 + 1 && Wo == (W + 2 - 3) / 2 + 1, "maxpool_fwd: bad output size");
    RowPlan p = plan_rows((int64_t)N * Ho * Wo, C);
    hipLaunchKernelGGL(k_maxpool_fwd, dim3(p.rowblocks, p.colblocks), dim3(256), 0, (hipStream_t)stream, x, N, H,
                       W, p.C4, y, yps, idx, Ho, Wo, p.CQ, p.RL);
    return check_launch("maxpool_fwd");
}

extern "C" int iswm_maxpool3x3s2_bwd(const float* dy, const uint8_t* idx, int N, int H, int W, int C, int Ho,
                                     int Wo, float* dx, iswm_stream_t stream) {
    ISWM_REQUIRE(dy && idx && dx && C % 4 == 0 && N > 0, "maxpool_bwd: bad argument");
    RowPlan p = plan_rows((int64_t)N * H * W, C);
    hipLaunchKernelGGL(k_maxpool_bwd, dim3(p.rowblocks, p.colblocks), dim3(256), 0, (hipStream_t)stream, dy, idx,
                       N, H, W, p.C4, Ho, Wo, dx, p.CQ, p.RL);
    return check_launch("maxpool_bwd");
}

extern "C" int iswm_gap_fwd(const float* x, int N, int HW, int C, int ldx, float* y, iswm_stream_t stream) {
    return iswm_gap_fwd_pl(x, 0, N, HW, C, ldx, y, stream);
}

extern "C" int iswm_gap_fwd_pl(const void* x, int64_t x_ps, int N, int HW, int C, int ldx, float* y, iswm_stream_t stream) {
    ISWM_REQUIRE(x && y && C % 4 == 0 && ldx % 4 == 0 && ldx >= C && N > 0 && HW > 0, "gap_fwd: bad argument");
    RowPlan p = plan_reduce(C);
    hipLaunchKernelGGL(k_gap_fwd, dim3(1, p.colblocks, N), dim3(256), 0, (hipStream_t)stream, x, x_ps, HW, p.C4, ldx, y,
                       p.CQ, p.RL);
    return check_launch("gap_fwd");
}

extern "C" int iswm_gap_bwd(const float* dy, int N, int HW, int C, float* dx, int lddx, int accumulate,
                            iswm_stream_t stream) {
    ISWM_REQUIRE(dy && dx && C % 4 == 0 && lddx % 4 == 0 && lddx >= C && N > 0 && HW > 0, "gap_bwd: bad argument");
    RowPlan p = plan_rows(HW, C);
    dim3 grid(p.rowblocks, p.colblocks, N);
    const float mul = 1.f / (float)HW;
    if (accumulate)
        hipLaunchKernelGGL((k_bcast<true>), grid, dim3(256), 0, (hipStream_t)stream, dy, HW, p.C4, mul, dx, lddx,
                           (int64_t)0, p.CQ, p.RL);
    else
        hipLaunchKernelGGL((k_bcast<false>), grid, dim3(256), 0, (hipStream_t)stream, dy, HW, p.C4, mul, dx, lddx,
                           (int64_t)0, p.CQ, p.RL);
    return check_launch("gap_bwd");
}

extern "C" int iswm_bcast_fwd(const float* v, int N, int HW, int C, float* y, int ldy, iswm_stream_t stream) {
    return iswm_bcast_fwd_pl(v, N, HW, C, y, ldy, 0, stream);
}

extern "C" int iswm_bcast_fwd_pl(const float* v, int N, int HW, int C, void* y, int ldy, int64_t y_ps, iswm_stream_t stream) {
    ISWM_REQUIRE(v && y && C % 4 == 0 && ldy % 4 == 0 && ldy >= C && N > 0 && HW > 0, "bcast_fwd: bad argument");
    RowPlan p = plan_rows(HW, C);
    hipLaunchKernelGGL((k_bcast<false>), dim3(p.rowblocks, p.colblocks, N), dim3(256), 0, (hipStream_t)stream, v,
                       HW, p.C4, 1.f, y, ldy, y_ps, p.CQ, p.RL);
    return check_launch("bcast_fwd");
}

extern "C" int iswm_bcast_bwd(const float* dy, int lddy, int N, int HW, int C, float* dv, iswm_stream_t stream) {
    ISWM_REQUIRE(dy && dv && C % 4 == 0 && lddy % 4 == 0 && lddy >= C && N > 0 && HW > 0, "bcast_bwd: bad argument");
    RowPlan p = plan_reduce(C);
    hipLaunchKernelGGL(k_bcast_bwd, dim3(1, p.colblocks, N), dim3(256), 0, (hipStream_t)stream, dy, HW, p.C4, lddy,
                       dv, p.CQ, p.RL);
    return check_launch("bcast_bwd");
}
```

### iswm_amd/csrc/rowmap.h

```cpp
#pragma once
#include "common.h"
#include "planes.h"

namespace iswm {

struct RowPlan {
    int C4;
    int CQ;
    int RL;
    int colblocks;
    int rowblocks;
};

inline RowPlan plan_rows(int64_t M, int C, int fixed_rowblocks = 0) {
    RowPlan p;
    p.C4 = C / 4;
    p.CQ = p.C4 < 256 ? p.C4 : 256;
    p.RL = 256 / p.CQ;
    p.colblocks = (p.C4 + p.CQ - 1) / p.CQ;
    if (fixed_rowblocks > 0) {
        p.rowblocks = fixed_rowblocks;
    } else {
        int64_t rb = (M + (int64_t)p.RL * 4 - 1) / ((int64_t)p.RL * 4);
        int64_t cap = 8192 / p.colblocks;
        if (cap < 1) cap = 1;
        if (rb > cap) rb = cap;
        if (rb < 1) rb = 1;
        p.rowblocks = (int)rb;
    }
    return p;
}

struct RowThread {
    int c4;
    int rl;
    bool active;
    int64_t row0;
    int64_t rstep;
};

__device__ __forceinline__ RowThread row_thread(int C4, int CQ, int RL) {
    RowThread r;
    const int t = threadIdx.x;
    r.rl = t / CQ;
    const int cq = t - r.rl * CQ;
    r.c4 = blockIdx.y * CQ + cq;
    r.active = (r.rl < RL) && (r.c4 < C4);
    r.row0 = (int64_t)blockIdx.x * RL + r.rl;
    r.rstep = (int64_t)gridDim.x * RL;
    return r;
}

__device__ __forceinline__ float4 ld4(const float* p) { return *reinterpret_cast<const float4*>(p); }
__device__ __forceinline__ void st4(float* p, float4 v) { *reinterpret_cast<float4*>(p) = v; }

}
```

### iswm_amd/network/_hip.py

```python

import torch
import torch.nn as nn

from .. import ops


MASK_RECORDER = None
POOL_RECORDER = None
CALIB_RECORDER = None


def pad4(c):
    return (c + 3) // 4 * 4


def pad_cin(c):
    if c % 32 == 0 or c < 128:
        return pad4(c)
    return (c + 31) // 32 * 32


def dense_flat(t):
    if t.dim() == 4 and not t.is_contiguous():
        v = t.permute(0, 2, 3, 1)
# ... 178 lines not shown
        if c < self.in_channels or c % 4 != 0:
            raise ValueError("depthwise conv over %d channels got a %d-channel buffer" % (self.in_channels, c))
        return ops.ConvGeom(x, c, self.kernel_size[0], self.kernel_size[1], self.stride[0], self.padding[0],
                            self.dilation[0])

    def fwd(self, x, save, out=None):
        g = self.geometry(x)
        y = ops.dwconv2d_fwd(x, self.weight.contiguous(), g, self.bias, out)
        self._saved = (x, g) if save else None
        return y

    def is_dw3x3(self):
        return (self.kernel_size[0] == 3 and self.stride[0] in (1, 2) and self.padding[0] == self.dilation[0] and
                self.bias is None)

    def fwd_stats(self, x, save, want_stats):
        g = self.geometry(x)
        y, partials, tiles = ops.dwconv3x3_fwd_stats(x, self.weight.contiguous(), g, want_stats)
        self._saved = (x, g) if save else None
        return y, partials, tiles

    def bwd_fused(self, dy, sink, need_dx=True, dx=None, accumulate=False):
        x, g = self._saved
        self._saved = None
        need_dw, buf, tgt = self.weight.requires_grad, None, None
        if need_dw:
            buf = sink.target(self.weight)
            tgt = buf if buf.is_contiguous() else None
        if not (need_dx or need_dw):
            return None
        dx, dw = ops.dwconv3x3_bwd(x, dy, self.weight.contiguous(), g, self.in_channels, dx, accumulate, tgt, need_dx, need_dw)
        if need_dw:
            if tgt is None:
                buf.copy_(dw)
            sink.done(self.weight)
        return dx

    def bwd(self, dy, sink, need_dx=True, dx=None, accumulate=False):
        x, g = self._saved
        self._saved = None
        _bias_grad(self.bias, dy, sink)
        if self.weight.requires_grad:
            buf = sink.target(self.weight)
            if buf.is_contiguous():
                ops.dwconv2d_wgrad(x, dy, g, self.in_channels, buf)
            else:
                buf.copy_(ops.dwconv2d_wgrad(x, dy, g, self.in_channels))
            sink.done(self.weight)
        if not need_dx:
            return None
        return ops.dwconv2d_dgrad(dy, self.weight.contiguous(), g, tuple(x.shape), dx, accumulate)

    def out_channels_of(self, cin):
        return self.out_channels


class BatchNorm2d(nn.BatchNorm2d):
    pass


class ReLU(nn.ReLU):
    pass


class ReLU6(nn.ReLU6):
    pass


class Dropout(HipModule, nn.Dropout):

    def __init__(self, *a, **k):
        nn.Dropout.__init__(self, *a, **k)
        self._calls = 0
        self._mask = None

    def fwd(self, x, save):
        if not self.training or self.p == 0.0:
            self._mask = None
            return x
        self._calls += 1
        y, mask = ops.dropout_fwd(x, self.p, torch.initial_seed() & 0x7FFFFFFFFFFFFFFF, self._calls)
        self._mask = mask if save else None
        return y

    def bwd(self, dy, sink):
        if self._mask is None:
            return dy
        dx = ops.dropout_bwd(dy.contiguous(), self._mask, self.p)
        self._mask = None
        return dx


def cba_fwd(conv, bn, relu, x, save, residual=None, out=None, out_fmt=None):
    sep = None
    if isinstance(conv, SeparableBase):
        sep, conv = conv, conv.body[1]
        x = sep.body[0].fwd(x, save)
    training = bn.training
    if bn.momentum is None or not bn.track_running_stats or not bn.affine:
        raise NotImplementedError("HIP BatchNorm2d supports affine=True, momentum!=None, running stats")
    if isinstance(conv, DepthwiseConv2d):
        g = conv.geometry(x)
        if conv.is_dw3x3():
            y, partials, tiles = conv.fwd_stats(x, save, training)
        else:
            y = conv.fwd(x, save)
            partials, tiles = _colstat_partials(y, training)
        return _cba_finish(conv, bn, relu, x, y, g, partials, tiles, training, save, residual, out, sep, True, out_fmt)
    g = conv.geometry(x)
    if conv.bias is None:
        y, partials, tiles = ops.conv2d_fwd(x, conv.weight_for(0), g, want_stats=training)
    else:
        y, _, _ = ops.conv2d_fwd(x, conv.weight_for(0), g, bias=conv.bias_p())
        partials, tiles = _colstat_partials(y, training)
    return _cba_finish(conv, bn, relu, x, y, g, partials, tiles, training, save, residual, out, sep, False, out_fmt)


def _colstat_partials(y, training):
    if not training:
        return None, (0, 0)
    partials, nt, tr = ops.colstat(y)
    return partials, (nt, tr)


def _bn_coef(bn, y, partials, tiles, training):
    if not training:
        return ops.bn_eval_coeffs(bn.weight, bn.bias, bn.running_mean, bn.running_var, bn.eps)
    count = y.shape[0] * y.shape[1] * y.shape[2]
    if count <= 1:
        raise ValueError("Expected more than 1 value per channel when training, got input size %s" % (tuple(y.shape),))
    coef = ops.bn_finalize(partials, tiles[0], count, tiles[1], bn.weight, bn.bias, bn.running_mean, bn.running_var,
                           bn.momentum, bn.eps)
    if not getattr(bn, "_iswm_nbt_fused", False):
        bn.num_batches_tracked.add_(1)
    return coef


def _bn_grad_targets(bn, sink):
    return [sink.target(p) if p.requires_grad else torch.empty_like(p) for p in (bn.weight, bn.bias)]


def _bn_grads_done(bn, sink):
    for p in (bn.weight, bn.bias):
        if p.requires_grad:
            sink.done(p)


def _cba_finish(conv, bn, relu, x, y, g, partials, tiles, training, save, residual, out, sep, dw, out_fmt=None):
    coef = _bn_coef(bn, y, partials, tiles, training)
    if out_fmt is None:
        want_planes = ops.planes_on() and y.shape[3] % 64 == 0
    else:
        want_planes = out_fmt == "planes" and ops.planes_on() and y.shape[3] % 64 == 0
    o = ops.bn_apply(y, coef, relu, residual, out, planes=want_planes)
    if MASK_RECORDER is not None and relu:
        of = ops.as_f32(o)
        MASK_RECORDER[bn] = (of > 0) & (of < 6) if relu == 6 and relu is not True else (of > 0)
    if CALIB_RECORDER is not None:
        CALIB_RECORDER.record(conv, o)
    ctx = None
    if save:
        ctx = dict(x=x, y=y, out=o, coef=coef, g=g, relu=relu, training=training, res=residual is not None, sep=sep, dw=dw)
    return o, ctx


_BN3_FUSE = True


def _bn_stats_request(up):
    if up is None or not ops.planes_on() or up.get("bn_stats") is not None:
        return None
    if ops._relu_code(up["relu"]) not in (0, 1):
        return None
    if up.get("res"):
        if not (_BN3_FUSE and ops._relu_code(up["relu"]) == 1 and ops.is_planes(up["out"]) and up["training"]):
            return None
        return ops.BnStats(up["y"], up["coef"], up["relu"], mask=up["out"])
    return ops.BnStats(up["y"], up["coef"], up["relu"])


def cba_bwd_bn(conv, bn, ctx, dout, sink, dy_out=None, need_dx=True):
    y, o = ctx["y"], ctx["out"]
    sep = ctx.get("sep")
    if sep is not None:
        conv = sep.body[1]
    gw = bn.weight
    dgamma, dbeta = _bn_grad_targets(bn, sink)
    dyp = (not ctx.get("dw")) and ops.planes_conv_ok(conv.cin_p, conv.cout_p, 1) and (need_dx or ops.is_planes(ctx["x"]))
    st = ctx.pop("bn_stats", None)
    if st is not None and st.partials is not None and st.masked:
        dout = ops.as_f32(dout)
        dy, _ = ops.bn_backward(dout, None, y, ctx["coef"], gw, False, ctx["training"], dgamma, dbeta, want_dres=False,
                                dy=dy_out, dy_planes=dyp, stats=st)
        dres = dout if ctx["res"] else None
    else:
        dy, dres = ops.bn_backward(ops.as_f32(dout), o if ctx["relu"] else None, y, ctx["coef"], gw, ctx["relu"], ctx["training"],
                                   dgamma, dbeta, want_dres=ctx["res"], dy=dy_out, dy_planes=dyp, stats=st)
    _bn_grads_done(bn, sink)
    return dy, dres


def cba_bwd(conv, bn, ctx, dout, sink, need_dx=True, dx=None, accumulate=False, up=None):
    x, g = ctx["x"], ctx["g"]
    sep = ctx.get("sep")
    dy, dres = cba_bwd_bn(conv, bn, ctx, dout, sink, need_dx=need_dx or sep is not None)
    if sep is not None:
        conv = sep.body[1]
    if ctx.get("dw"):
        if conv.is_dw3x3():
            return conv.bwd_fused(dy, sink, need_dx, dx, accumulate), dres
        return conv.bwd(dy, sink, need_dx, dx, accumulate), dres
    conv.write_wgrad(x, dy, g, sink)
    _bias_grad(conv.bias, dy, sink)
    if sep is not None:
        dmid = ops.conv2d_dgrad(dy, conv.weight_for(1), g, tuple(x.shape))
        return sep.body[0].bwd(dmid, sink, need_dx, dx, accumulate), dres
    if need_dx:
        req = _bn_stats_request(up) if (up is not None and tuple(up["y"].shape) == tuple(x.shape)) else None
        dx = ops.conv2d_dgrad(dy, conv.weight_for(1), g, tuple(x.shape), dx, accumulate, bn_stats=req)
        if req is not None and req.partials is not None:
            up["bn_stats"] = req
    else:
        dx = None
    return dx, dres


def fuse_batch_counters(root):
    bns = [m for m in root.modules() if isinstance(m, nn.BatchNorm2d) and m.num_batches_tracked is not None]
    if not bns:
        return None
    flat = torch.stack([m.num_batches_tracked.detach().reshape(()) for m in bns]).contiguous()
    for i, m in enumerate(bns):
        m._buffers["num_batches_tracked"] = flat[i]
        m._iswm_nbt_fused = True
    return flat


class WeightPacker(object):

    def __init__(self, root):
        self.convs = [m for m in root.modules() if isinstance(m, Conv2d) and not m.needs_pack()]
        self.key, self.jobs, self.njobs, self.blocks, self.entries = None, None, 0, 0, []

    def _build(self, dev):
        import ctypes
        from .. import _lib
        lib = _lib.load()
        jobs, entries, first = [], [], 0
        keep = []
        for m in self.convs:
            w = m.weight
            v = w.permute(0, 2, 3, 1)
            if not (w.is_cuda and v.is_contiguous()):
                continue
            taps = m.kernel_size[0] * m.kernel_size[1]
            bufs = {}
            kinds = []
            for kind in (0, 1):
                if ops.planes_on() and lib.iswm_packed_weight_bytes(m.out_channels, taps, m.in_channels, kind + 2):
                    kinds.append(kind + 2)
                else:
                    kinds.append(kind)
            for kind in kinds:
                nb = lib.iswm_packed_weight_bytes(m.out_channels, taps, m.in_channels, kind)
                if nb == 0:
                    continue
                buf = torch.empty((nb // 4,), dtype=torch.float32, device=dev)
                bufs[kind] = buf
                jobs.append((w.data_ptr(), buf.data_ptr(), m.out_channels, taps, m.in_channels, kind, first, 0))
                first += lib.iswm_pack_job_blocks(m.out_channels, taps, m.in_channels, kind)
            if bufs:
                e = dict(live=False, epoch=-1, version=-1, ptr=w.data_ptr(), buf={k: bufs.get(k) for k in range(4)})
                m._iswm_wpk = e
                entries.append((m, e))
                keep.append(bufs)

        class _Job(ctypes.Structure):
            _fields_ = [("w", ctypes.c_void_p), ("packed", ctypes.c_void_p), ("Cout", ctypes.c_int), ("taps", ctypes.c_int),
                        ("Cin", ctypes.c_int), ("kind", ctypes.c_int), ("first_block", ctypes.c_int),
                        ("reserved", ctypes.c_int)]
        arr = (_Job * max(1, len(jobs)))()
        for i, j in enumerate(jobs):
            arr[i] = _Job(*j)
        self.jobs = torch.frombuffer(bytearray(bytes(arr)), dtype=torch.uint8).to(dev) if jobs else None
        self.njobs, self.blocks, self.entries = len(jobs), first, entries

    def begin(self):
        from .. import _lib
        math = _lib.load().iswm_get_conv_math()
        if math < 1 or not ops._USE_PACKED or not self.convs:
            return
        key = (math, ops.planes_on()) + tuple(m.weight.data_ptr() for m in self.convs)
        if key != self.key:
            self._build(self.convs[0].weight.device)
            self.key = key
        if self.njobs == 0:
            return
        ops.call("iswm_pack_weights_batch", ops._p(self.jobs), self.njobs, self.blocks, ops._stream())
        for m, e in self.entries:
            e["live"], e["epoch"], e["version"] = True, ops.WEIGHTS_EPOCH, m.weight._version

    def end(self):
        for _, e in self.entries:
            e["live"] = False


_CLS_FUSE = True


def cls_fusable(conv, bn, relu, cls):
    return (_CLS_FUSE and CALIB_RECORDER is None and relu is True and type(conv) is Conv2d and conv.out_channels == 256 and
            conv.bias is None and type(cls) is Conv2d and cls.in_channels == 256 and cls.out_channels <= 4 and
            tuple(cls.kernel_size) == (1, 1) and tuple(cls.stride) == (1, 1) and tuple(cls.padding) == (0, 0) and
            bn.momentum is not None and bn.track_running_stats and bn.affine)


# ... 117 lines not shown
```

### iswm_amd/network/backbone/resnet.py

```python
import torch
import torch.nn as nn

from .. import _hip
from ..._hip_compat import FloatFunctional
from ... import ops

__all__ = ['ResNet', 'resnet50', 'resnet101', 'resnet152']


def conv3x3(in_planes, out_planes, stride=1, groups=1, dilation=1):
    return _hip.Conv2d(in_planes, out_planes, kernel_size=3, stride=stride, padding=dilation, groups=groups,
                       bias=False, dilation=dilation)


def conv1x1(in_planes, out_planes, stride=1):
    return _hip.Conv2d(in_planes, out_planes, kernel_size=1, stride=stride, bias=False)


class Bottleneck(_hip.HipModule):
    expansion = 4

    def __init__(self, inplanes, planes, stride=1, downsample=None, groups=1, base_width=64, dilation=1,
                 norm_layer=None):
        super(Bottleneck, self).__init__()
        if norm_layer is None:
            norm_layer = _hip.BatchNorm2d
        width = int(planes * (base_width / 64.)) * groups
        self.conv1 = conv1x1(inplanes, width)
        self.bn1 = norm_layer(width)
        self.conv2 = conv3x3(width, width, stride, groups, dilation)
        self.bn2 = norm_layer(width)
        self.conv3 = conv1x1(width, planes * self.expansion)
        self.bn3 = norm_layer(planes * self.expansion)
        self.relu = _hip.ReLU(inplace=True)
        self.downsample = downsample
        self.stride = stride
        self.add = FloatFunctional()
        self._saved = None

    def fwd(self, x, save):
        o1, c1 = _hip.cba_fwd(self.conv1, self.bn1, True, x, save)
        o2, c2 = _hip.cba_fwd(self.conv2, self.bn2, True, o1, save)
        identity, cd = x, None
        if self.downsample is not None:
            identity, cd = _hip.cba_fwd(self.downsample[0], self.downsample[1], False, x, save)
        out, c3 = _hip.cba_fwd(self.conv3, self.bn3, True, o2, save, residual=identity)
        self._saved = (c1, c2, c3, cd) if save else None
        return out

    def bwd(self, dout, sink, need_dx=True, up=None, dx0=None):
        c1, c2, c3, cd = self._saved
        self._saved = None
        d2, dres = _hip.cba_bwd(self.conv3, self.bn3, c3, dout, sink, up=c2)
        d1, _ = _hip.cba_bwd(self.conv2, self.bn2, c2, d2, sink, up=c1)
        if cd is not None:
            dx, _ = _hip.cba_bwd(self.conv1, self.bn1, c1, d1, sink, dx=dx0, accumulate=dx0 is not None)
            dx, _ = _hip.cba_bwd(self.downsample[0], self.downsample[1], cd, dres, sink, dx=dx, accumulate=True)
        else:
            dx, _ = _hip.cba_bwd(self.conv1, self.bn1, c1, d1, sink, dx=dres, accumulate=True, up=up)
            if dx0 is not None:
                dx = ops.add_inplace(dx, dx0)
        return dx

    def out_channels_of(self, cin):
        return self.conv3.out_channels


class _Layer(_hip.HipModule, nn.Sequential):
    accepts_dx0 = True

    def fwd(self, x, save):
        for m in self:
            x = m.fwd(x, save)
        return x

    def bwd(self, dy, sink, dx0=None):
        blocks = list(self)
        for i in range(len(blocks) - 1, -1, -1):
            up = None
            if i > 0 and blocks[i].downsample is None and blocks[i - 1]._saved is not None:
                up = blocks[i - 1]._saved[2]
            dy = blocks[i].bwd(dy, sink, up=up, dx0=dx0 if i == 0 else None)
        return dy

    def out_channels_of(self, cin):
        return list(self)[-1].conv3.out_channels


class MaxPool2d(_hip.HipModule, nn.MaxPool2d):

    def fwd(self, x, save):
        if (self.kernel_size, self.stride, self.padding) != (3, 2, 1):
            raise NotImplementedError("HIP max-pool is the stem's 3x3 / stride 2 / pad 1")
        y, idx = ops.maxpool_fwd(x, planes=ops.planes_on() and x.shape[3] % 64 == 0)
        if _hip.POOL_RECORDER is not None:
            _hip.POOL_RECORDER[self] = idx
        if _hip.CALIB_RECORDER is not None:
            _hip.CALIB_RECORDER.record(self, y)
        self._saved = (idx, tuple(x.shape)) if save else None
        return y

    def bwd(self, dy, sink):
        idx, shape = self._saved
        self._saved = None
        return ops.maxpool_bwd(dy, idx, shape)


class ResNet(_hip.HipModule):

    def __init__(self, block, layers, num_classes=1000, zero_init_residual=False, groups=1, width_per_group=64,
                 replace_stride_with_dilation=None, norm_layer=None):
        super(ResNet, self).__init__()
        if norm_layer is None:
            norm_layer = _hip.BatchNorm2d
        self._norm_layer = norm_layer
        if groups != 1 or width_per_group != 64:
            raise NotImplementedError("HIP backbone covers the groups=1 / width 64 family (resnet50/101/152)")
        self.inplanes = 64
        self.dilation = 1
        if replace_stride_with_dilation is None:
            replace_stride_with_dilation = [False, False, False]
        if len(replace_stride_with_dilation) != 3:
            raise ValueError("replace_stride_with_dilation should be None "
                             "or a 3-element tuple, got {}".format(replace_stride_with_dilation))
        self.groups = groups
        self.base_width = width_per_group
        self.conv1 = _hip.Conv2d(3, self.inplanes, kernel_size=7, stride=2, padding=3, bias=False)
        self.bn1 = norm_layer(self.inplanes)
        self.relu = _hip.ReLU(inplace=True)
        self.maxpool = MaxPool2d(kernel_size=3, stride=2, padding=1)
        self.layer1 = self._make_layer(block, 64, layers[0])
        self.layer2 = self._make_layer(block, 128, layers[1], stride=2, dilate=replace_stride_with_dilation[0])
        self.layer3 = self._make_layer(block, 256, layers[2], stride=2, dilate=replace_stride_with_dilation[1])
        self.layer4 = self._make_layer(block, 512, layers[3], stride=2, dilate=replace_stride_with_dilation[2])
        self.avgpool = nn.AdaptiveAvgPool2d((1, 1))
        self.fc = nn.Linear(512 * block.expansion, num_classes)

        for m in self.modules():
            if isinstance(m, nn.Conv2d):
                nn.init.kaiming_normal_(m.weight, mode='fan_out', nonlinearity='relu')
            elif isinstance(m, (nn.BatchNorm2d, nn.GroupNorm)):
                nn.init.constant_(m.weight, 1)
                nn.init.constant_(m.bias, 0)
        if zero_init_residual:
            for m in self.modules():
                if isinstance(m, Bottleneck):
                    nn.init.constant_(m.bn3.weight, 0)

    def _make_layer(self, block, planes, blocks, stride=1, dilate=False):
        norm_layer = self._norm_layer
        downsample = None
        previous_dilation = self.dilation
        if dilate:
            self.dilation *= stride
            stride = 1
        if stride != 1 or self.inplanes != planes * block.expansion:
            downsample = nn.Sequential(
                conv1x1(self.inplanes, planes * block.expansion, stride),
                norm_layer(planes * block.expansion),
            )
        layers = [block(self.inplanes, planes, stride, downsample, self.groups, self.base_width,
                        previous_dilation, norm_layer)]
        self.inplanes = planes * block.expansion
        for _ in range(1, blocks):
            layers.append(block(self.inplanes, planes, groups=self.groups, base_width=self.base_width,
                                dilation=self.dilation, norm_layer=norm_layer))
        return _Layer(*layers)

    def forward(self, x):
        raise NotImplementedError("the ImageNet classification head (avgpool+fc) is not on the segmentation hot "
                                  "path; wrap the backbone in network.utils.IntermediateLayerGetter")


def _resnet(arch, block, layers, pretrained, progress, **kwargs):
    model = ResNet(block, layers, **kwargs)
    if pretrained:
        raise RuntimeError("pretrained=True needs a download; load a checkpoint with load_state_dict instead")
    return model


def resnet50(pretrained=False, progress=True, **kwargs):
    return _resnet('resnet50', Bottleneck, [3, 4, 6, 3], pretrained, progress, **kwargs)


def resnet101(pretrained=False, progress=True, **kwargs):
    return _resnet('resnet101', Bottleneck, [3, 4, 23, 3], pretrained, progress, **kwargs)


def resnet152(pretrained=False, progress=True, **kwargs):
    return _resnet('resnet152', Bottleneck, [3, 8, 36, 3], pretrained, progress, **kwargs)
```

### iswm_amd/network/utils.py

```python
from collections import OrderedDict

import torch
import torch.nn as nn

from . import _hip
from .. import ops
from .._hip_compat import DeQuantStub, QuantStub


class _SegBridge(torch.autograd.Function):

    @staticmethod
    def forward(ctx, model, x, *params):
        ctx.model = model
        ctx.need_dx = x.requires_grad
        ctx.cin = x.shape[1]
        return model._fwd(x, True)

    @staticmethod
    def backward(ctx, dlogits):
        dx = ctx.model._bwd(dlogits.contiguous(), ctx.need_dx)
        return (None, dx) + (None,) * (len(ctx.needs_input_grad) - 2)


class _SimpleSegmentationModel(nn.Module):
    def __init__(self, backbone, classifier):
        super(_SimpleSegmentationModel, self).__init__()
        self.backbone = backbone
        self.classifier = classifier
        self.quant = QuantStub()
        self.dequant = DeQuantStub()
        self._saved = None
        self._iswm_on_ready = None

    def _counters(self):
        flat = getattr(self, "_iswm_nbt", None)
        first = next((m for m in self.modules() if isinstance(m, nn.BatchNorm2d)), None)
        if first is None:
            return None
        nbt = first.num_batches_tracked
        if flat is None or flat.device != nbt.device or nbt.data_ptr() != flat.data_ptr():
            flat = _hip.fuse_batch_counters(self)
            object.__setattr__(self, "_iswm_nbt", flat)
        return flat

    def _packer(self):
        pk = getattr(self, "_iswm_packer", None)
        if pk is None:
            pk = _hip.WeightPacker(self)
            object.__setattr__(self, "_iswm_packer", pk)
        return pk

    def _fwd(self, x, save):
        h, w = x.shape[2:]
        yl = self._fwd_lowres(x, save)
        nc = self.classifier.num_classes
        return ops.bilinear_to_nchw_fwd(yl, nc, h, w)

    def _fwd_lowres(self, x, save):
        c = x.shape[1]
        if self.training:
            flat = self._counters()
            if flat is not None:
                bns = [m for m in self.modules() if isinstance(m, nn.BatchNorm2d)]
                if all(b.training for b in bns):
                    flat.add_(1)
                else:
                    for b in bns:
                        if b.training and b.num_batches_tracked is not None:
                            b.num_batches_tracked.add_(1)
        pk = self._packer()
        pk.begin()
        try:
            xh = ops.nchw_to_nhwc(x)
            feats = self.backbone.fwd(xh, save)
            yl = self.classifier.fwd(feats, save)
        except BaseException:
            pk.end()
            raise
        if not save:
            pk.end()
        self._saved = (tuple(yl.shape), c) if save else None
        return yl

    def _bwd(self, dlogits, need_dx):
        (n, hl, wl, cp), cin = self._saved
        self._saved = None
        sink = _hip.GradSink(self._iswm_on_ready)
        try:
            dyl = ops.bilinear_to_nchw_bwd(dlogits, hl, wl, cp)
            dfeats = self.classifier.bwd(dyl, sink)
            if getattr(self, "_debug_keep_dfeats", False):
                self._debug_dfeats = {k: v.clone() for k, v in dfeats.items()}
            dxh = self.backbone.bwd(dfeats, sink, need_dx)
        finally:
            self._packer().end()
        return ops.nhwc_to_nchw(dxh, cin) if need_dx else None

    def forward(self, x):
        if not (torch.is_tensor(x) and x.is_cuda and x.dtype == torch.float32 and x.dim() == 4):
            raise ValueError("iswm_amd model takes a 4-D fp32 CUDA NCHW tensor (there is no CPU fallback)")
        if torch.is_grad_enabled():
            params = [p for p in self.parameters() if p.requires_grad]
            if params or x.requires_grad:
                return _SegBridge.apply(self, x, *params)
        return self._fwd(x, False)

    def forward_lowres(self, x):
        if not (torch.is_tensor(x) and x.is_cuda and x.dtype == torch.float32 and x.dim() == 4):
            raise ValueError("iswm_amd model takes a 4-D fp32 CUDA NCHW tensor (there is no CPU fallback)")
        if torch.is_grad_enabled() and (x.requires_grad or any(p.requires_grad for p in self.parameters())):
            raise RuntimeError("forward_lowres has no backward: call it under torch.no_grad()")
        return ops.as_f32(self._fwd_lowres(x, False))


class IntermediateLayerGetter(nn.ModuleDict):

    def __init__(self, model, return_layers, hrnet_flag=False):
        if not set(return_layers).issubset([name for name, _ in model.named_children()]):
            raise ValueError("return_layers are not present in model")
        if hrnet_flag:
            raise NotImplementedError("HRNet backbones are not part of this build")
        self.hrnet_flag = hrnet_flag
        orig_return_layers = return_layers
        return_layers = {k: v for k, v in return_layers.items()}
        layers = OrderedDict()
        for name, module in model.named_children():
            layers[name] = module
            if name in return_layers:
                del return_layers[name]
            if not return_layers:
                break
        super(IntermediateLayerGetter, self).__init__(layers)
        self.return_layers = orig_return_layers
        self._saved = None

    def fwd(self, x, save):
        out = OrderedDict()
        stem_ctx = None
        for name, module in self.named_children():
            if name == "conv1":
                fmt = "f32" if "maxpool" in self._modules else None
                x, stem_ctx = _hip.cba_fwd(self["conv1"], self["bn1"], True, x, save, out_fmt=fmt)
            elif name in ("bn1", "relu"):
                pass
            else:
                x = module.fwd(x, save)
            if name in self.return_layers:
                out[self.return_layers[name]] = x
        self._saved = stem_ctx if save else None
        return out

    def bwd(self, dfeats, sink, need_dx=False):
        names = [n for n, _ in self.named_children()]
        inv = {v: k for k, v in self.return_layers.items()}
        tap = {inv[k]: g for k, g in dfeats.items() if g is not None}
        dy = None
        order = list(reversed(names))
        for k, name in enumerate(order):
            if name in tap:
                g = tap.pop(name)
                dy = g if dy is None else ops.add_inplace(dy, g)
            if name in ("relu", "bn1"):
                continue
            if name == "conv1":
                dy, _ = _hip.cba_bwd(self["conv1"], self["bn1"], self._saved, dy, sink, need_dx=need_dx)
            else:
                below = order[k + 1] if k + 1 < len(order) else None
                if below in tap and getattr(self[name], "accepts_dx0", False) and not ops.is_planes(tap[below]):
                    dy = self[name].bwd(dy, sink, dx0=tap.pop(below))
                elif below is None and isinstance(self[name], _hip.HipSequential):
                    dy = self[name].bwd(dy, sink, need_dx=need_dx)
                else:
                    dy = self[name].bwd(dy, sink)
        self._saved = None
        return dy

    def forward(self, x):
        feats = self.fwd(ops.nchw_to_nhwc(x), False)
        return OrderedDict((k, ops.nhwc_to_nchw(v)) for k, v in feats.items())
```

### iswm_amd/ops.py

```python
import collections
import ctypes
import functools

import numpy as np
import torch

from . import _lib
from ._lib import ConvDesc, call

BN_EPS = 1e-5


def _stream():
    return ctypes.c_void_p(torch.cuda.current_stream().cuda_stream)


def _p(t):
    return ctypes.c_void_p(t.data_ptr()) if t is not None else None


def geom(t, dtype=torch.float32):
    if isinstance(t, Planes):
        raise ValueError("this operation takes an fp32 NHWC tensor, not Planes (use .f32())")
    if t.dim() != 4 or t.dtype != dtype or not t.is_cuda:
# ... 503 lines not shown
    _, n, h, w, ctot, ld, ps = xgeom(dyc)
    nb = len(ksize)
    assert ctot >= nb * cout
    plan = aspp_plan(n, h, w, cin, cout, ksize, dil, 1, dyc.device)
    if plan is None:
        return None
    if dx is None:
        assert not accumulate
        dx = new_act(n, h, w, cin, dyc.device)
    d = aspp_desc(n, h, w, cin, cout, geom(dx)[4], cout)
    gs = []
    for k, dl in zip(ksize, dil):
        g = ConvGeom(dx, cout, k, k, 1, dl * (k - 1) // 2, dl)
        g.alg_cin, g.alg_cout = cin, cout
        gs.append(g)
    px, xps, pdw, ws, need = None, 0, None, None, 0
    if dws is not None:
        px, xps = x.t, pgeom(x)[5]
        pdw = _ptr_array(dws)
        lib = _lib.load()
        for k, dl in zip(ksize, dil):
            db = ConvDesc(n, h, w, cin, h, w, cout, k, k, 1, dl * (k - 1) // 2, dl, pgeom(x)[4], ld)
            need = max(need, lib.iswm_conv2d_wgrad_planes_workspace(ctypes.byref(db)))
        ws = torch.empty((max(need, 16) // 4,), dtype=torch.float32, device=dyc.device)
        d = aspp_desc(n, h, w, cin, cout, pgeom(x)[4], cout)
        assert geom(dx)[4] == pgeom(x)[4], "iswm_aspp_bwd takes ONE pitch for x and dx"
    with _timed("k_conv_pl2t<true>", gs):
        call("iswm_aspp_bwd", ctypes.byref(d), nb, _int_array(ksize), _int_array(dil), _p(plan), _p(dyc.t), ps, ld, _ptr_array(wpks),
             _p(dx), int(bool(accumulate)), _p(px), xps, pdw, _p(ws), need, _stream())
    return dx


def dwconv2d_fwd(x, w, g, bias=None, out=None):
    x = as_f32(x)
    ldx = geom(x)[4]
    if out is None:
        out = new_act(g.n, g.ho, g.wo, g.cin, x.device)
    d = g.desc(ldx, geom(out)[4])
    call("iswm_dwconv2d_fwd", ctypes.byref(d), _p(x), _p(w), w.shape[0], _p(bias), _p(out), _stream())
    return out


def dwconv2d_dgrad(dy, w, g, x_like_shape, dx=None, accumulate=False):
    if dx is None:
        assert not accumulate
        dx = new_act(*x_like_shape, dy.device)
    d = g.desc(geom(dx)[4], geom(dy)[4])
    call("iswm_dwconv2d_dgrad", ctypes.byref(d), _p(dy), _p(w), w.shape[0], _p(dx), int(bool(accumulate)), _stream())
    return dx


def dwconv2d_wgrad(x, dy, g, cw, dw=None):
    x, dy = as_f32(x), as_f32(dy)
    if dw is None:
        dw = torch.empty((cw, 1, g.kh, g.kw), dtype=torch.float32, device=x.device)
    d = g.desc(geom(x)[4], geom(dy)[4])
    need = _lib.load().iswm_dwconv2d_wgrad_workspace(ctypes.byref(d))
    ws = torch.empty((need // 8,), dtype=torch.float64, device=x.device)
    call("iswm_dwconv2d_wgrad", ctypes.byref(d), _p(x), _p(dy), cw, _p(dw), _p(ws), need, _stream())
    return dw


def dwconv3x3_fwd_stats(x, w, g, want_stats, out=None):
    x = as_f32(x)
    if out is None:
        out = new_act(g.n, g.ho, g.wo, g.cin, x.device)
    d = g.desc(geom(x)[4], geom(out)[4])
    partials, tiles = None, (0, 0)
    if want_stats:
        lib = _lib.load()
        tiles = (lib.iswm_dwconv3x3_stat_tiles(ctypes.byref(d)), lib.iswm_dwconv3x3_stat_tile_rows(ctypes.byref(d)))
        partials = torch.empty((2, tiles[0], g.cin), dtype=torch.float32, device=x.device)
    call("iswm_dwconv3x3_fwd_stats", ctypes.byref(d), _p(x), _p(w), w.shape[0], _p(out), _p(partials), _stream())
    return out, partials, tiles


def dwconv3x3_bwd(x, dy, w, g, cw, dx=None, accumulate=False, dw=None, need_dx=True, need_dw=True):
    x, dy = as_f32(x), as_f32(dy)
    if need_dx and dx is None:
        assert not accumulate
        dx = new_act(*x.shape, dy.device)
    if not need_dx:
        dx = None
    d = g.desc(geom(x)[4], geom(dy)[4])
    lddx = geom(dx)[4] if dx is not None else 0
    ws, need = None, 0
    if need_dw:
        if dw is None:
            dw = torch.empty((cw, 1, 3, 3), dtype=torch.float32, device=x.device)
        need = _lib.load().iswm_dwconv3x3_bwd_workspace(ctypes.byref(d))
        ws = torch.empty((need // 4,), dtype=torch.float32, device=x.device)
    else:
        dw = None
    call("iswm_dwconv3x3_bwd", ctypes.byref(d), _p(x), _p(dy), _p(w), cw, _p(dx), lddx, int(bool(accumulate)), _p(dw), _p(ws),
         need, _stream())
    return dx, dw


def rows(t):
    n, h, w, c, ld = geom(t)
    return n * h * w, c, ld


def xrows(t):
    p, n, h, w, c, ld, ps = xgeom(t)
    return p, n * h * w, c, ld, ps


def colstat(x):
    m, c, ld = rows(x)
    tile_rows = _lib.load().iswm_colstat_tile_rows(m)
    tiles = (m + tile_rows - 1) // tile_rows
    partials = torch.empty((3, tiles, c), dtype=torch.float32, device=x.device)
    call("iswm_colstat_res", _p(x), m, c, ld, _p(partials), _stream())
    return partials, tiles, tile_rows


def bn_finalize(partials, tiles, count, tile_rows, gamma, beta, running_mean, running_var, momentum, eps=BN_EPS):
    c = partials.shape[2]
    coef = torch.empty((4, c), dtype=torch.float32, device=partials.device)
    name = "iswm_bn_finalize_res" if (partials.dim() == 3 and partials.shape[0] == 3) else "iswm_bn_finalize"
    call(name, _p(partials), tiles, c, count, tile_rows, _p(gamma), _p(beta), _p(running_mean),
         _p(running_var), float(momentum), float(eps), _p(coef[0]), _p(coef[1]), _p(coef[2]), _p(coef[3]), _stream())
    return coef


def bn_eval_coeffs(gamma, beta, running_mean, running_var, eps=BN_EPS):
    c = running_mean.numel()
    coef = torch.empty((4, c), dtype=torch.float32, device=running_mean.device)
    call("iswm_bn_eval_coeffs", c, _p(gamma), _p(beta), _p(running_mean), _p(running_var), float(eps), _p(coef[0]),
         _p(coef[1]), _p(coef[2]), _p(coef[3]), _stream())
    return coef


def _relu_code(relu):
    return 6 if (relu == 6 and relu is not True) else int(bool(relu))


def bn_apply(y, coef, relu, residual=None, out=None, planes=False):
    m, c, ldy = rows(y)
    if out is None:
        out = new_planes(*y.shape, y.device) if planes else torch.empty(y.shape, dtype=torch.float32, device=y.device)
    po, mo, co, ldo, pso = xrows(out)
    assert (mo, co) == (m, c)
    pr, ldr, psr = None, 0, 0
    if residual is not None:
        pr, mr, cr, ldr, psr = xrows(residual)
        assert (mr, cr) == (m, c)
    call("iswm_bn_apply_pl", _p(y), m, c, ldy, _p(coef[0]), _p(coef[1]), _p(coef[2]), _p(pr), ldr, psr, _relu_code(relu),
         _p(po), ldo, pso, _stream())
    return out


def bn_backward(dout, out, y, coef, gamma, relu, training, dgamma, dbeta, want_dres=False, dy=None, dy_planes=False,
                stats=None):
    m, c, ldy = rows(y)
    _, _, ldd = rows(dout)
    po, ldo, pso = None, 0, 0
    if out is not None:
        po, _, _, ldo, pso = xrows(out)
    need = _lib.load().iswm_bn_bwd_workspace(m, c)
    ws = torch.empty((need // 8,), dtype=torch.float64, device=y.device)
    if dy is None:
        dy = new_planes(*y.shape, y.device) if dy_planes else torch.empty(y.shape, dtype=torch.float32, device=y.device)
    pdy, _, _, lddy, psdy = xrows(dy)
    dres = torch.empty(y.shape, dtype=torch.float32, device=y.device) if want_dres else None
    masky = _relu_code(relu) == 1 and not want_dres
    if stats is not None and stats.partials is not None:
        call("iswm_bn_backward_stats_pl", _p(dout), ldd, _p(po), ldo, pso, _p(y), ldy, m, c, _p(coef[2]), _p(coef[3]), _p(gamma),
             _p(coef[0]) if masky else None, _p(coef[1]) if masky else None,
             _relu_code(relu), int(bool(training)), _p(dgamma), _p(dbeta), _p(pdy), lddy, psdy, _p(dres),
             rows(dres)[2] if dres is not None else 0, _p(stats.partials), stats.tiles, _p(ws), need, _stream())
        return dy, dres
    call("iswm_bn_backward_pl", _p(dout), ldd, _p(po), ldo, pso, _p(y), ldy, m, c, _p(coef[2]), _p(coef[3]), _p(gamma),
         _p(coef[0]) if masky else None, _p(coef[1]) if masky else None,
         _relu_code(relu), int(bool(training)), _p(dgamma), _p(dbeta), _p(pdy), lddy, psdy, _p(dres),
         rows(dres)[2] if dres is not None else 0, _p(ws), need, _stream())
    return dy, dres


def bn_apply_classify(y, coef, wc4, bias4):
    m, c, ldy = rows(y)
    out = torch.empty(tuple(y.shape[:3]) + (4,), dtype=torch.float32, device=y.device)
    call("iswm_bn_apply_classify", _p(y), m, c, ldy, _p(coef[0]), _p(coef[1]), _p(coef[2]), _p(wc4), _p(bias4), _p(out), 4, _stream())
    return out


def bn_backward_classify(dlogit, wc4, y, coef, gamma, training, dgamma, dbeta, dy_planes):
    m, c, ldy = rows(y)
    _, cl, ldl = rows(dlogit)
    assert cl == 4
    need = _lib.load().iswm_bn_classify_bwd_workspace(m, c)
    ws = torch.empty((need // 8,), dtype=torch.float64, device=y.device)
    dy = new_planes(*y.shape, y.device) if dy_planes else torch.empty(y.shape, dtype=torch.float32, device=y.device)
    pdy, _, _, lddy, psdy = xrows(dy)
    dwc4 = torch.empty((4, c), dtype=torch.float32, device=y.device)
    call("iswm_bn_backward_classify", _p(dlogit), ldl, _p(wc4), _p(y), ldy, m, c, _p(coef[2]), _p(coef[3]), _p(gamma), _p(coef[0]),
         _p(coef[1]), int(bool(training)), _p(dgamma), _p(dbeta), _p(dwc4), _p(pdy), lddy, psdy, _p(ws), need, _stream())
    return dy, dwc4


def colsum(x):
    x = as_f32(x)
    partials, tiles, _ = colstat(x)
    c = x.shape[3]
    out = torch.empty((2, c), dtype=torch.float32, device=x.device)
    call("iswm_colsum_finalize", _p(partials), tiles, c, _p(out[0]), _p(out[1]), _stream())
    return out[0]


def maxpool_fwd(x, planes=False):
    x = as_f32(x)
    n, h, w, c, ld = geom(x)
    assert ld == c
    ho, wo = (h + 2 - 3) // 2 + 1, (w + 2 - 3) // 2 + 1
    y = new_planes(n, ho, wo, c, x.device) if planes else new_act(n, ho, wo, c, x.device)
    py, _, _, _, _, _, ps = xgeom(y)
    idx = torch.empty((n, ho, wo, c), dtype=torch.uint8, device=x.device)
    call("iswm_maxpool3x3s2_fwd_pl", _p(x), n, h, w, c, _p(py), ps, _p(idx), ho, wo, _stream())
    return y, idx


def maxpool_bwd(dy, idx, in_shape):
    n, h, w, c = in_shape
    _, ho, wo, _, ld = geom(dy)
    assert ld == c
    dx = new_act(n, h, w, c, dy.device)
    call("iswm_maxpool3x3s2_bwd", _p(dy), _p(idx), n, h, w, c, ho, wo, _p(dx), _stream())
    return dx


def gap_fwd(x):
    px, n, h, w, c, ld, ps = xgeom(x)
    y = new_act(n, 1, 1, c, x.device)
    call("iswm_gap_fwd_pl", _p(px), ps, n, h * w, c, ld, _p(y), _stream())
    return y


def gap_bwd(dy, dx, accumulate):
    n, h, w, c, ld = geom(dx)
    call("iswm_gap_bwd", _p(dy), n, h * w, c, _p(dx), ld, int(bool(accumulate)), _stream())
    return dx


def bcast_fwd(v, out):
    po, n, h, w, c, ld, ps = xgeom(out)
    call("iswm_bcast_fwd_pl", _p(as_f32(v)), n, h * w, c, _p(po), ld, ps, _stream())
    return out


def bcast_bwd(dy):
    n, h, w, c, ld = geom(dy)
    dv = new_act(n, 1, 1, c, dy.device)
    call("iswm_bcast_bwd", _p(dy), ld, n, h * w, c, _p(dv), _stream())
    return dv


def bilinear_fwd(x, ho, wo, out=None):
    x = as_f32(x)
    n, hi, wi, c, ldx = geom(x)
    if out is None:
        out = new_act(n, ho, wo, c, x.device)
    po, _, _, _, _, ldy, ps = xgeom(out)
    call("iswm_bilinear_fwd_pl", _p(x), n, hi, wi, c, ldx, _p(po), ps, ho, wo, ldy, _stream())
    return out


def bilinear_bwd(dy, hi, wi):
    n, ho, wo, c, lddy = geom(dy)
    dx = new_act(n, hi, wi, c, dy.device)
    call("iswm_bilinear_bwd", _p(dy), n, hi, wi, c, lddy, ho, wo, _p(dx), c, _stream())
    return dx


def bilinear_to_nchw_fwd(x, c, ho, wo):
    x = as_f32(x)
    n, hi, wi, cp, ldx = geom(x)
    y = torch.empty((n, c, ho, wo), dtype=torch.float32, device=x.device)
    call("iswm_bilinear_nhwc_to_nchw_fwd", _p(x), n, hi, wi, c, ldx, _p(y), ho, wo, _stream())
    return y


def bilinear_to_nchw_bwd(dy, hi, wi, cp):
    n, c, ho, wo = dy.shape
    assert dy.is_contiguous() and dy.dtype == torch.float32
    dx = new_act(n, hi, wi, cp, dy.device)
    call("iswm_bilinear_nhwc_to_nchw_bwd", _p(dy), n, hi, wi, c, cp, ho, wo, _p(dx), _stream())
    return dx


def nchw_to_nhwc(x, cp=None):
    assert x.dim() == 4 and x.dtype == torch.float32 and x.is_cuda
    x = x.contiguous()
    n, c, h, w = x.shape
    cp = cp or (c + 3) // 4 * 4
    y = new_act(n, h, w, cp, x.device)
    call("iswm_nchw_to_nhwc", _p(x), n, c, h * w, _p(y), cp, _stream())
    return y


def nhwc_to_nchw(x, c=None):
    x = as_f32(x)
    n, h, w, cc, ld = geom(x)
    c = c or cc
    y = torch.empty((n, c, h, w), dtype=torch.float32, device=x.device)
    call("iswm_nhwc_to_nchw", _p(x), n, c, h * w, ld, _p(y), _stream())
# ... 657 lines not shown
```

Before: 277.8 images/sec.

## Fuse stem BN+ReLU+maxpool and downsample BN into residual apply

Adds a fused kernel that applies BN, ReLU and 3x3/s2 maxpool to the stem conv output in one pass, and a backward kernel that scatters the pool gradient and runs the BN backward reduce/apply directly from the pool indices. It also defers the downsample branch's BN and folds it into the bottleneck's final BN+residual+ReLU kernel. Together these remove the full-resolution stem activation write/read and the separate downsample BN output tensor. The cost is more complex templated kernels, with the ReLU mask recomputed from y and the BN coefficients instead of being read from a stored output.

```diff
diff --git a/include/iswm_hip.h b/include/iswm_hip.h
--- a/include/iswm_hip.h
+++ b/include/iswm_hip.h
@@ -65,6 +65,17 @@
 int iswm_maxpool3x3s2_fwd_pl(const float* x, int N, int H, int W, int C, void* y, int64_t y_ps, uint8_t* idx, int Ho,
                              int Wo, iswm_stream_t stream);
 int iswm_gap_fwd_pl(const void* x, int64_t x_ps, int N, int HW, int C, int ldx, float* y, iswm_stream_t stream);
+int iswm_bn_relu_maxpool3x3s2_fwd_pl(const float* y, int N, int H, int W, int C, const float* scale, const float* shift,
+                                     const float* mean, void* out, int64_t out_ps, uint8_t* idx, int Ho, int Wo,
+                                     iswm_stream_t stream);
+int iswm_bn_backward_maxpool(const float* dpool, const uint8_t* idx, int N, int H, int W, int Ho, int Wo, const float* y,
+                             int ldy, int C, const float* mean, const float* invstd, const float* gamma,
+                             const float* mask_scale, const float* mask_shift, int training, float* dgamma, float* dbeta,
+                             void* dy, int lddy, int64_t dy_ps, void* workspace, size_t workspace_bytes,
+                             iswm_stream_t stream);
+int iswm_bn_apply_res_bn_pl(const float* y, int64_t M, int C, int ldy, const float* scale, const float* shift,
+                            const float* mean, const float* yr, int ldyr, const float* scale_r, const float* shift_r,
+                            const float* mean_r, int relu, void* out, int ldo, int64_t out_ps, iswm_stream_t stream);
 int iswm_bcast_fwd_pl(const float* v, int N, int HW, int C, void* y, int ldy, int64_t y_ps, iswm_stream_t stream);
 int iswm_bilinear_fwd_pl(const float* x, int N, int Hi, int Wi, int C, int ldx, void* y, int64_t y_ps, int Ho, int Wo,
                          int ldy, iswm_stream_t stream);
diff --git a/iswm_amd/_lib.py b/iswm_amd/_lib.py
--- a/iswm_amd/_lib.py
+++ b/iswm_amd/_lib.py
@@ -66,6 +66,10 @@
                                     c_int, c_int64, P, c_int, P, c_size_t, P]),
     "iswm_maxpool3x3s2_fwd_pl": (c_int, [P, c_int, c_int, c_int, c_int, P, c_int64, P, c_int, c_int, P]),
     "iswm_gap_fwd_pl": (c_int, [P, c_int64, c_int, c_int, c_int, c_int, P, P]),
+    "iswm_bn_relu_maxpool3x3s2_fwd_pl": (c_int, [P, c_int, c_int, c_int, c_int, P, P, P, P, c_int64, P, c_int, c_int, P]),
+    "iswm_bn_backward_maxpool": (c_int, [P, P, c_int, c_int, c_int, c_int, c_int, P, c_int, c_int, P, P, P, P, P, c_int, P, P,
+                                         P, c_int, c_int64, P, c_size_t, P]),
+    "iswm_bn_apply_res_bn_pl": (c_int, [P, c_int64, c_int, c_int, P, P, P, P, c_int, P, P, P, c_int, P, c_int, c_int64, P]),
     "iswm_bcast_fwd_pl": (c_int, [P, c_int, c_int, c_int, P, c_int, c_int64, P]),
     "iswm_bilinear_fwd_pl": (c_int, [P, c_int, c_int, c_int, c_int, c_int, P, c_int64, c_int, c_int, c_int, P]),
     "iswm_conv2d_pl2_weight_bytes": (c_size_t, [POINTER(ConvDesc), c_int]),
diff --git a/iswm_amd/csrc/bn.hip b/iswm_amd/csrc/bn.hip
--- a/iswm_amd/csrc/bn.hip
+++ b/iswm_amd/csrc/bn.hip
@@ -1,6 +1,6 @@
 #include <stdlib.h>
 
-#include "rowmap.h"
+#include "pool_window.h"
 
 namespace iswm {
 
@@ -214,9 +214,7 @@
     const float4 sc = ld4(scale + c), sh = ld4(shift + c), mu = ld4(mean + c);
     for (int64_t r = rt.row0; r < M; r += rt.rstep) {
         float4 v = ld4(y + r * ldy + c);
-        float4 o;
-        o.x = (v.x - mu.x) * sc.x + sh.x; o.y = (v.y - mu.y) * sc.y + sh.y;
-        o.z = (v.z - mu.z) * sc.z + sh.z; o.w = (v.w - mu.w) * sc.w + sh.w;
+        float4 o = bn_fwd4(v, mu, sc, sh);
         if (RES) {
             float4 q = ld4x(res, r * ldr + c, rps);
             o.x += q.x; o.y += q.y; o.z += q.z; o.w += q.w;
@@ -242,11 +240,7 @@
     const float4 sc0 = ld4(scale + c), sc1 = ld4(scale + c + 4), sh0 = ld4(shift + c), sh1 = ld4(shift + c + 4);
     const float4 mu0 = ld4(mean + c), mu1 = ld4(mean + c + 4);
     auto one = [&](int64_t r, const float4 v0, const float4 v1, const float4 q0, const float4 q1) {
-        float4 o0, o1;
-        o0.x = (v0.x - mu0.x) * sc0.x + sh0.x; o0.y = (v0.y - mu0.y) * sc0.y + sh0.y;
-        o0.z = (v0.z - mu0.z) * sc0.z + sh0.z; o0.w = (v0.w - mu0.w) * sc0.w + sh0.w;
-        o1.x = (v1.x - mu1.x) * sc1.x + sh1.x; o1.y = (v1.y - mu1.y) * sc1.y + sh1.y;
-        o1.z = (v1.z - mu1.z) * sc1.z + sh1.z; o1.w = (v1.w - mu1.w) * sc1.w + sh1.w;
+        float4 o0 = bn_fwd4(v0, mu0, sc0, sh0), o1 = bn_fwd4(v1, mu1, sc1, sh1);
         if (RES) {
             o0.x += q0.x; o0.y += q0.y; o0.z += q0.z; o0.w += q0.w;
             o1.x += q1.x; o1.y += q1.y; o1.z += q1.z; o1.w += q1.w;
@@ -283,15 +277,87 @@
     }
 }
 
-template <int RELU, bool DBL>
-__global__ __launch_bounds__(256) void k_bn_bwd_reduce(const float* __restrict__ dout, int ldd,
-                                                       const void* __restrict__ out, int ldo, int64_t ops,
-                                                       const float* __restrict__ y, int ldy, int64_t M,
-                                                       int C4, int C, const float* __restrict__ mean,
-                                                       const float* __restrict__ invstd,
-                                                       const float* __restrict__ mscale,
-                                                       const float* __restrict__ mshift, int CQ, int RL,
-                                                       int tiles, double* __restrict__ partials) {
+template <int RELU>
+__device__ __forceinline__ float4 add_act4(float4 o, const float4 q) {
+    o.x += q.x; o.y += q.y; o.z += q.z; o.w += q.w;
+    if (RELU) {
+        o.x = fmaxf(o.x, 0.f); o.y = fmaxf(o.y, 0.f); o.z = fmaxf(o.z, 0.f); o.w = fmaxf(o.w, 0.f);
+    }
+    if (RELU == 2) {
+        o.x = fminf(o.x, 6.f); o.y = fminf(o.y, 6.f); o.z = fminf(o.z, 6.f); o.w = fminf(o.w, 6.f);
+    }
+    return o;
+}
+
+template <int RELU>
+__global__ __launch_bounds__(256) void k_bn_apply_res_bn(const float* __restrict__ y, int64_t M, int C4, int ldy,
+                                                         const float* __restrict__ scale, const float* __restrict__ shift,
+                                                         const float* __restrict__ mean, const float* __restrict__ yr,
+                                                         int ldyr, const float* __restrict__ scale_r,
+                                                         const float* __restrict__ shift_r, const float* __restrict__ mean_r,
+                                                         void* __restrict__ out, int ldo, int64_t ops, int CQ, int RL) {
+    RowThread rt = row_thread(C4, CQ, RL);
+    if (!rt.active) return;
+    const int c = rt.c4 * 4;
+    const float4 sc = ld4(scale + c), sh = ld4(shift + c), mu = ld4(mean + c);
+    const float4 scr = ld4(scale_r + c), shr = ld4(shift_r + c), mur = ld4(mean_r + c);
+    for (int64_t r = rt.row0; r < M; r += rt.rstep) {
+        const float4 v = ld4(y + r * ldy + c), vr = ld4(yr + r * ldyr + c);
+        st4x(out, r * ldo + c, ops, add_act4<RELU>(bn_fwd4(v, mu, sc, sh), bn_fwd4(vr, mur, scr, shr)));
+    }
+}
+
+template <int RELU>
+__global__ __launch_bounds__(256) void k_bn_apply_res_bn8(const float* __restrict__ y, int64_t M, int C8, int ldy,
+                                                          const float* __restrict__ scale, const float* __restrict__ shift,
+                                                          const float* __restrict__ mean, const float* __restrict__ yr,
+                                                          int ldyr, const float* __restrict__ scale_r,
+                                                          const float* __restrict__ shift_r, const float* __restrict__ mean_r,
+                                                          void* __restrict__ out, int ldo, int64_t ops, int CQ, int RL) {
+    RowThread rt = row_thread(C8, CQ, RL);
+    if (!rt.active) return;
+    const int c = rt.c4 * 8;
+    const float4 sc0 = ld4(scale + c), sc1 = ld4(scale + c + 4), sh0 = ld4(shift + c), sh1 = ld4(shift + c + 4);
+    const float4 mu0 = ld4(mean + c), mu1 = ld4(mean + c + 4);
+    const float4 scr0 = ld4(scale_r + c), scr1 = ld4(scale_r + c + 4), shr0 = ld4(shift_r + c), shr1 = ld4(shift_r + c + 4);
+    const float4 mur0 = ld4(mean_r + c), mur1 = ld4(mean_r + c + 4);
+    auto one = [&](int64_t r, const float4 v0, const float4 v1, const float4 w0, const float4 w1) {
+        st8x(out, r * ldo + c, ops, add_act4<RELU>(bn_fwd4(v0, mu0, sc0, sh0), bn_fwd4(w0, mur0, scr0, shr0)),
+             add_act4<RELU>(bn_fwd4(v1, mu1, sc1, sh1), bn_fwd4(w1, mur1, scr1, shr1)));
+    };
+    int64_t r = rt.row0;
+    for (; r + rt.rstep < M; r += 2 * rt.rstep) {
+        const int64_t r2 = r + rt.rstep;
+        const float4 a0 = ld4(y + r * ldy + c), a1 = ld4(y + r * ldy + c + 4);
+        const float4 b0 = ld4(y + r2 * ldy + c), b1 = ld4(y + r2 * ldy + c + 4);
+        const float4 ra0 = ld4(yr + r * ldyr + c), ra1 = ld4(yr + r * ldyr + c + 4);
+        const float4 rb0 = ld4(yr + r2 * ldyr + c), rb1 = ld4(yr + r2 * ldyr + c + 4);
+        one(r, a0, a1, ra0, ra1);
+        one(r2, b0, b1, rb0, rb1);
+    }
+    if (r < M) {
+        const float4 a0 = ld4(y + r * ldy + c), a1 = ld4(y + r * ldy + c + 4);
+        const float4 ra0 = ld4(yr + r * ldyr + c), ra1 = ld4(yr + r * ldyr + c + 4);
+        one(r, a0, a1, ra0, ra1);
+    }
+}
+
+__device__ __forceinline__ float4 relu_gate(const float4 g, const float4 z) {
+    return make_float4(z.x > 0.f ? g.x : 0.f, z.y > 0.f ? g.y : 0.f, z.z > 0.f ? g.z : 0.f, z.w > 0.f ? g.w : 0.f);
+}
+
+struct DoutRows {
+    const float* p;
+    int ld;
+    __device__ __forceinline__ float4 operator()(int64_t r, int c) const { return ld4(p + r * ld + c); }
+};
+
+template <int RELU, bool DBL, typename Dout>
+__device__ __forceinline__ void bn_bwd_reduce_rows(const Dout& dout, const void* __restrict__ out, int ldo, int64_t ops,
+                                                   const float* __restrict__ y, int ldy, int64_t M, int C4, int C,
+                                                   const float* __restrict__ mean, const float* __restrict__ invstd,
+                                                   const float* __restrict__ mscale, const float* __restrict__ mshift,
+                                                   int CQ, int RL, int tiles, double* __restrict__ partials) {
     __shared__ double red[2 * 256 * 4];
     RowThread rt = row_thread(C4, CQ, RL);
     double s[4] = {0, 0, 0, 0}, s2[4] = {0, 0, 0, 0};
@@ -309,7 +375,7 @@
             for (int u = 0; u < 8; ++u) {
                 const int64_t rr = r + u * rt.rstep;
                 if (rr < M) {
-                    float4 g = ld4(dout + rr * ldd + c);
+                    float4 g = dout(rr, c);
                     float4 v = ld4(y + rr * ldy + c);
                     if (RELU == 1) {
                         float4 o = ld4x_hi(out, rr * ldo + c, ops);
@@ -320,10 +386,7 @@
                         g.x = (o.x > 0.f && o.x < 6.f) ? g.x : 0.f; g.y = (o.y > 0.f && o.y < 6.f) ? g.y : 0.f;
                         g.z = (o.z > 0.f && o.z < 6.f) ? g.z : 0.f; g.w = (o.w > 0.f && o.w < 6.f) ? g.w : 0.f;
                     } else if (RELU == 2) {
-                        g.x = (v.x - mu.x) * msc.x + msh.x > 0.f ? g.x : 0.f;
-                        g.y = (v.y - mu.y) * msc.y + msh.y > 0.f ? g.y : 0.f;
-                        g.z = (v.z - mu.z) * msc.z + msh.z > 0.f ? g.z : 0.f;
-                        g.w = (v.w - mu.w) * msc.w + msh.w > 0.f ? g.w : 0.f;
+                        g = relu_gate(g, bn_fwd4(v, mu, msc, msh));
                     }
                     if (DBL) {
                         const double gd[4] = {g.x, g.y, g.z, g.w}, vd[4] = {v.x, v.y, v.z, v.w};
@@ -367,6 +430,29 @@
             partials[(size_t)(tiles + blockIdx.x) * C + rt.c4 * 4 + k] = s2[k];
         }
     }
+}
+
+template <int RELU, bool DBL>
+__global__ __launch_bounds__(256) void k_bn_bwd_reduce(const float* __restrict__ dout, int ldd,
+                                                       const void* __restrict__ out, int ldo, int64_t ops,
+                                                       const float* __restrict__ y, int ldy, int64_t M,
+                                                       int C4, int C, const float* __restrict__ mean,
+                                                       const float* __restrict__ invstd,
+                                                       const float* __restrict__ mscale,
+                                                       const float* __restrict__ mshift, int CQ, int RL,
+                                                       int tiles, double* __restrict__ partials) {
+    bn_bwd_reduce_rows<RELU, DBL>(DoutRows{dout, ldd}, out, ldo, ops, y, ldy, M, C4, C, mean, invstd, mscale, mshift, CQ, RL,
+                                  tiles, partials);
+}
+
+template <bool DBL>
+__global__ __launch_bounds__(256) void k_bn_bwd_reduce_pool(PoolGradRows dout, const float* __restrict__ y, int ldy, int64_t M,
+                                                            int C4, int C, const float* __restrict__ mean,
+                                                            const float* __restrict__ invstd,
+                                                            const float* __restrict__ mscale,
+                                                            const float* __restrict__ mshift, int CQ, int RL, int tiles,
+                                                            double* __restrict__ partials) {
+    bn_bwd_reduce_rows<2, DBL>(dout, nullptr, 0, 0, y, ldy, M, C4, C, mean, invstd, mscale, mshift, CQ, RL, tiles, partials);
 }
 
 template <typename T, int CPB>
@@ -407,6 +493,65 @@
     }
 }
 
+template <int RELU, bool TRAIN, bool DRES, typename Dout>
+__device__ __forceinline__ void bn_bwd_apply_rows(const Dout& dout, const void* __restrict__ out, int ldo, int64_t ops,
+                                                  const float* __restrict__ y, int ldy, int64_t M, int C4, int C,
+                                                  const float* __restrict__ mean, const float* __restrict__ invstd,
+                                                  const float* __restrict__ gamma, const float* __restrict__ mscale,
+                                                  const float* __restrict__ mshift, const double* __restrict__ sums,
+                                                  double inv_count, void* __restrict__ dy, int lddy, int64_t dyps,
+                                                  float* __restrict__ dres, int lddres, int CQ, int RL) {
+    RowThread rt = row_thread(C4, CQ, RL);
+    if (!rt.active) return;
+    const int c = rt.c4 * 4;
+    const float4 mu = ld4(mean + c), is = ld4(invstd + c);
+    const float4 ga = gamma ? ld4(gamma + c) : make_float4(1.f, 1.f, 1.f, 1.f);
+    const double mud[4] = {mu.x, mu.y, mu.z, mu.w}, isd[4] = {is.x, is.y, is.z, is.w};
+    const double gi[4] = {(double)ga.x * is.x, (double)ga.y * is.y, (double)ga.z * is.z, (double)ga.w * is.w};
+    float4 msc = make_float4(0.f, 0.f, 0.f, 0.f), msh = msc;
+    if (RELU == 2) {
+        msc = ld4(mscale + c);
+        msh = ld4(mshift + c);
+    }
+    double k1[4] = {0, 0, 0, 0}, k2[4] = {0, 0, 0, 0};
+    if (TRAIN) {
+#pragma unroll
+        for (int k = 0; k < 4; ++k) {
+            k1[k] = sums[c + k] * inv_count;
+            k2[k] = sums[C + c + k] * inv_count;
+        }
+    }
+    for (int64_t r = rt.row0; r < M; r += rt.rstep) {
+        float4 g = dout(r, c);
+        float4 v = make_float4(0.f, 0.f, 0.f, 0.f);
+        if (TRAIN || RELU == 2) v = ld4(y + r * ldy + c);
+        if (RELU == 1) {
+            float4 o = ld4x_hi(out, r * ldo + c, ops);
+            g.x = o.x > 0.f ? g.x : 0.f; g.y = o.y > 0.f ? g.y : 0.f;
+            g.z = o.z > 0.f ? g.z : 0.f; g.w = o.w > 0.f ? g.w : 0.f;
+        } else if (RELU == 3) {
+            float4 o = ld4x_hi(out, r * ldo + c, ops);
+            g.x = (o.x > 0.f && o.x < 6.f) ? g.x : 0.f; g.y = (o.y > 0.f && o.y < 6.f) ? g.y : 0.f;
+            g.z = (o.z > 0.f && o.z < 6.f) ? g.z : 0.f; g.w = (o.w > 0.f && o.w < 6.f) ? g.w : 0.f;
+        } else if (RELU == 2) {
+            g = relu_gate(g, bn_fwd4(v, mu, msc, msh));
+        }
+        if (DRES) st4(dres + r * lddres + c, g);
+        const double gd[4] = {g.x, g.y, g.z, g.w};
+        float d[4];
+        if (TRAIN) {
+            const double vd[4] = {v.x, v.y, v.z, v.w};
+#pragma unroll
+            for (int k = 0; k < 4; ++k)
+                d[k] = (float)(gi[k] * (gd[k] - k1[k] - (vd[k] - mud[k]) * isd[k] * k2[k]));
+        } else {
+#pragma unroll
+            for (int k = 0; k < 4; ++k) d[k] = (float)(gi[k] * gd[k]);
+        }
+        st4x(dy, r * lddy + c, dyps, make_float4(d[0], d[1], d[2], d[3]));
+    }
+}
+
 template <int RELU, bool TRAIN, bool DRES>
 __global__ __launch_bounds__(256) void k_bn_bwd_apply(const float* __restrict__ dout, int ldd,
                                                       const void* __restrict__ out, int ldo, int64_t ops,
@@ -419,58 +564,21 @@
                                                       const double* __restrict__ sums, double inv_count,
                                                       void* __restrict__ dy, int lddy, int64_t dyps,
                                                       float* __restrict__ dres, int lddres, int CQ, int RL) {
-    RowThread rt = row_thread(C4, CQ, RL);
-    if (!rt.active) return;
-    const int c = rt.c4 * 4;
-    const float4 mu = ld4(mean + c), is = ld4(invstd + c);
-    const float4 ga = gamma ? ld4(gamma + c) : make_float4(1.f, 1.f, 1.f, 1.f);
-    const double mud[4] = {mu.x, mu.y, mu.z, mu.w}, isd[4] = {is.x, is.y, is.z, is.w};
-    const double gi[4] = {(double)ga.x * is.x, (double)ga.y * is.y, (double)ga.z * is.z, (double)ga.w * is.w};
-    float4 msc = make_float4(0.f, 0.f, 0.f, 0.f), msh = msc;
-    if (RELU == 2) {
-        msc = ld4(mscale + c);
-        msh = ld4(mshift + c);
-    }
-    double k1[4] = {0, 0, 0, 0}, k2[4] = {0, 0, 0, 0};
-    if (TRAIN) {
-#pragma unroll
-        for (int k = 0; k < 4; ++k) {
-            k1[k] = sums[c + k] * inv_count;
-            k2[k] = sums[C + c + k] * inv_count;
-        }
-    }
-    for (int64_t r = rt.row0; r < M; r += rt.rstep) {
-        float4 g = ld4(dout + r * ldd + c);
-        float4 v = make_float4(0.f, 0.f, 0.f, 0.f);
-        if (TRAIN || RELU == 2) v = ld4(y + r * ldy + c);
-        if (RELU == 1) {
-            float4 o = ld4x_hi(out, r * ldo + c, ops);
-            g.x = o.x > 0.f ? g.x : 0.f; g.y = o.y > 0.f ? g.y : 0.f;
-            g.z = o.z > 0.f ? g.z : 0.f; g.w = o.w > 0.f ? g.w : 0.f;
-        } else if (RELU == 3) {
-            float4 o = ld4x_hi(out, r * ldo + c, ops);
-            g.x = (o.x > 0.f && o.x < 6.f) ? g.x : 0.f; g.y = (o.y > 0.f && o.y < 6.f) ? g.y : 0.f;
-            g.z = (o.z > 0.f && o.z < 6.f) ? g.z : 0.f; g.w = (o.w > 0.f && o.w < 6.f) ? g.w : 0.f;
-        } else if (RELU == 2) {
-            g.x = (v.x - mu.x) * msc.x + msh.x > 0.f ? g.x : 0.f;
-            g.y = (v.y - mu.y) * msc.y + msh.y > 0.f ? g.y : 0.f;
-            g.z = (v.z - mu.z) * msc.z + msh.z > 0.f ? g.z : 0.f;
-            g.w = (v.w - mu.w) * msc.w + msh.w > 0.f ? g.w : 0.f;
-        }
-        if (DRES) st4(dres + r * lddres + c, g);
-        const double gd[4] = {g.x, g.y, g.z, g.w};
-        float d[4];
-        if (TRAIN) {
-            const double vd[4] = {v.x, v.y, v.z, v.w};
-#pragma unroll
-            for (int k = 0; k < 4; ++k)
-                d[k] = (float)(gi[k] * (gd[k] - k1[k] - (vd[k] - mud[k]) * isd[k] * k2[k]));
-        } else {
-#pragma unroll
-            for (int k = 0; k < 4; ++k) d[k] = (float)(gi[k] * gd[k]);
-        }
-        st4x(dy, r * lddy + c, dyps, make_float4(d[0], d[1], d[2], d[3]));
-    }
+    bn_bwd_apply_rows<RELU, TRAIN, DRES>(DoutRows{dout, ldd}, out, ldo, ops, y, ldy, M, C4, C, mean, invstd, gamma, mscale,
+                                         mshift, sums, inv_count, dy, lddy, dyps, dres, lddres, CQ, RL);
+}
+
+template <bool TRAIN>
+__global__ __launch_bounds__(256) void k_bn_bwd_apply_pool(PoolGradRows dout, const float* __restrict__ y, int ldy, int64_t M,
+                                                           int C4, int C, const float* __restrict__ mean,
+                                                           const float* __restrict__ invstd,
+                                                           const float* __restrict__ gamma,
+                                                           const float* __restrict__ mscale,
+                                                           const float* __restrict__ mshift,
+                                                           const double* __restrict__ sums, double inv_count,
+                                                           void* __restrict__ dy, int lddy, int64_t dyps, int CQ, int RL) {
+    bn_bwd_apply_rows<2, TRAIN, false>(dout, nullptr, 0, 0, y, ldy, M, C4, C, mean, invstd, gamma, mscale, mshift, sums,
+                                       inv_count, dy, lddy, dyps, nullptr, 0, CQ, RL);
 }
 
 static int chk_rows(const char* what, int64_t M, int C, int ld) {
@@ -618,6 +726,43 @@
     else LAUNCH(0, false);
 #undef LAUNCH
     return check_launch("bn_apply");
+}
+
+extern "C" int iswm_bn_apply_res_bn_pl(const float* y, int64_t M, int C, int ldy, const float* scale, const float* shift,
+                                       const float* mean, const float* yr, int ldyr, const float* scale_r,
+                                       const float* shift_r, const float* mean_r, int relu, void* out, int ldo,
+                                       int64_t out_ps, iswm_stream_t stream) {
+    if (int e = chk_rows("bn_apply_res_bn", M, C, ldy)) return e;
+    if (int e = chk_rows("bn_apply_res_bn(yr)", M, C, ldyr)) return e;
+    ISWM_REQUIRE(y && scale && shift && mean && yr && scale_r && shift_r && mean_r && out && ldo % 4 == 0 && ldo >= C,
+                 "bn_apply_res_bn: bad argument");
+    ISWM_REQUIRE(aligned16(y) && aligned16(yr), "bn_apply_res_bn: misaligned tensor");
+    ISWM_REQUIRE(relu == 0 || relu == 1 || relu == 6, "bn_apply_res_bn: relu must be 0 (none), 1 (ReLU) or 6 (ReLU6)");
+    if (int e = chk_ps("bn_apply_res_bn(out)", out, M, ldo, out_ps)) return e;
+    hipStream_t s = (hipStream_t)stream;
+    if (out_ps != 0 && C % 8 == 0 && ldy % 8 == 0 && ldo % 8 == 0 && aligned16(out) && (out_ps < 0 || out_ps % 8 == 0) &&
+        ldyr % 8 == 0) {
+        RowPlan p = plan_rows(M, C / 2);
+        dim3 grid(p.rowblocks, p.colblocks), blk(256);
+#define LAUNCH8(R)                                                                                                         \
+    hipLaunchKernelGGL((k_bn_apply_res_bn8<R>), grid, blk, 0, s, y, M, p.C4, ldy, scale, shift, mean, yr, ldyr, scale_r, \
+                       shift_r, mean_r, out, ldo, out_ps, p.CQ, p.RL)
+        if (relu == 6) LAUNCH8(2);
+        else if (relu) LAUNCH8(1);
+        else LAUNCH8(0);
+#undef LAUNCH8
+        return check_launch("bn_apply_res_bn8");
+    }
+    RowPlan p = plan_rows(M, C);
+    dim3 grid(p.rowblocks, p.colblocks), blk(256);
+#define LAUNCH(R)                                                                                                         \
+    hipLaunchKernelGGL((k_bn_apply_res_bn<R>), grid, blk, 0, s, y, M, p.C4, ldy, scale, shift, mean, yr, ldyr, scale_r, \
+                       shift_r, mean_r, out, ldo, out_ps, p.CQ, p.RL)
+    if (relu == 6) LAUNCH(2);
+    else if (relu) LAUNCH(1);
+    else LAUNCH(0);
+#undef LAUNCH
+    return check_launch("bn_apply_res_bn");
 }
 
 extern "C" size_t iswm_bn_bwd_workspace(int64_t M, int C) {
@@ -736,6 +881,59 @@
                             tiles, stream);
 }
 
+extern "C" int iswm_bn_backward_maxpool(const float* dpool, const uint8_t* idx, int N, int H, int W, int Ho, int Wo,
+                                        const float* y, int ldy, int C, const float* mean, const float* invstd,
+                                        const float* gamma, const float* mask_scale, const float* mask_shift, int training,
+                                        float* dgamma, float* dbeta, void* dy, int lddy, int64_t dy_ps, void* workspace,
+                                        size_t workspace_bytes, iswm_stream_t stream) {
+    ISWM_REQUIRE(N > 0 && H > 0 && W > 0 && Ho == (H + 2 - 3) / 2 + 1 && Wo == (W + 2 - 3) / 2 + 1,
+                 "bn_backward_maxpool: bad map size");
+    const int64_t M = (int64_t)N * H * W;
+    ISWM_REQUIRE(M <= INT32_MAX, "bn_backward_maxpool: map of 2^31 pixels or more");
+    if (int e = chk_rows("bn_backward_maxpool", M, C, ldy)) return e;
+    if (int e = chk_ps("bn_backward_maxpool(dy)", dy, M, lddy, dy_ps)) return e;
+    ISWM_REQUIRE(dpool && idx && y && mean && invstd && mask_scale && mask_shift && dgamma && dbeta && dy && workspace,
+                 "bn_backward_maxpool: null pointer");
+    ISWM_REQUIRE(aligned16(dpool) && aligned16(y) && (reinterpret_cast<uintptr_t>(idx) & 3) == 0,
+                 "bn_backward_maxpool: misaligned tensor");
+    ISWM_REQUIRE(lddy % 4 == 0 && lddy >= C, "bn_backward_maxpool: bad pitch");
+    ISWM_REQUIRE(workspace_bytes >= iswm_bn_bwd_workspace(M, C) && aligned16(workspace),
+                 "bn_backward_maxpool: workspace too small");
+    const int tiles = iswm_colstat_tiles(M);
+    double* partials = (double*)workspace;
+    double* sums = partials + (size_t)2 * tiles * C;
+    hipStream_t s = (hipStream_t)stream;
+    const PoolGradRows dout = {dpool, idx, H, W, Ho, Wo, C};
+    {
+        RowPlan p = plan_rows(M, C, tiles);
+        dim3 grid(p.rowblocks, p.colblocks), blk(256);
+        if (M <= 8192)
+            hipLaunchKernelGGL((k_bn_bwd_reduce_pool<true>), grid, blk, 0, s, dout, y, ldy, M, p.C4, C, mean, invstd, mask_scale,
+                               mask_shift, p.CQ, p.RL, tiles, partials);
+        else
+            hipLaunchKernelGGL((k_bn_bwd_reduce_pool<false>), grid, blk, 0, s, dout, y, ldy, M, p.C4, C, mean, invstd,
+                               mask_scale, mask_shift, p.CQ, p.RL, tiles, partials);
+        if (int e = check_launch("bn_bwd_reduce_pool")) return e;
+    }
+    if (tiles > 32)
+        hipLaunchKernelGGL((k_bn_bwd_finalize<double, 4>), dim3((C + 3) / 4), dim3(256), 0, s, partials, tiles, C, dgamma,
+                           dbeta, sums);
+    else
+        hipLaunchKernelGGL((k_bn_bwd_finalize<double, 16>), dim3((C + 15) / 16), dim3(256), 0, s, partials, tiles, C, dgamma,
+                           dbeta, sums);
+    if (int e = check_launch("bn_bwd_finalize")) return e;
+    const double inv = 1.0 / (double)M;
+    RowPlan p = plan_rows(M, C);
+    dim3 grid(p.rowblocks, p.colblocks), blk(256);
+    if (training)
+        hipLaunchKernelGGL((k_bn_bwd_apply_pool<true>), grid, blk, 0, s, dout, y, ldy, M, p.C4, C, mean, invstd, gamma,
+                           mask_scale, mask_shift, sums, inv, dy, lddy, dy_ps, p.CQ, p.RL);
+    else
+        hipLaunchKernelGGL((k_bn_bwd_apply_pool<false>), grid, blk, 0, s, dout, y, ldy, M, p.C4, C, mean, invstd, gamma,
+                           mask_scale, mask_shift, sums, inv, dy, lddy, dy_ps, p.CQ, p.RL);
+    return check_launch("bn_bwd_apply_pool");
+}
+
 extern "C" int iswm_colsum_finalize(const float* partials, int tiles, int C, float* out, float* scratch,
                                     iswm_stream_t stream) {
     ISWM_REQUIRE(partials && out && scratch && tiles > 0 && C > 0, "colsum_finalize: bad argument");
diff --git a/iswm_amd/csrc/pool.hip b/iswm_amd/csrc/pool.hip
--- a/iswm_amd/csrc/pool.hip
+++ b/iswm_amd/csrc/pool.hip
@@ -1,42 +1,54 @@
-#include "rowmap.h"
+#include "pool_window.h"
 
 namespace iswm {
 
-__global__ __launch_bounds__(256) void k_maxpool_fwd(const float* __restrict__ x, int N, int H, int W, int C4,
-                                                     void* __restrict__ y, int64_t yps, uint8_t* __restrict__ idx, int Ho,
-                                                     int Wo, int CQ, int RL) {
-    RowThread rt = row_thread(C4, CQ, RL);
-    if (!rt.active) return;
+struct PoolTapPlain {
+    __device__ __forceinline__ float4 operator()(const float4 v) const { return v; }
+};
+
+struct PoolTapBnRelu {
+    float4 mu, sc, sh;
+    __device__ __forceinline__ float4 operator()(const float4 v) const {
+        const float4 o = bn_fwd4(v, mu, sc, sh);
+        return make_float4(fmaxf(o.x, 0.f), fmaxf(o.y, 0.f), fmaxf(o.z, 0.f), fmaxf(o.w, 0.f));
+    }
+};
+
+template <typename Tap>
+__device__ __forceinline__ void maxpool_fwd_rows(const RowThread& rt, const float* __restrict__ x, int N, int H, int W, int C4,
+                                                 const Tap& tap, void* __restrict__ y, int64_t yps,
+                                                 uint8_t* __restrict__ idx, int Ho, int Wo) {
     const int C = C4 * 4, c = rt.c4 * 4;
     const int64_t Mo = (int64_t)N * Ho * Wo;
     for (int64_t r = rt.row0; r < Mo; r += rt.rstep) {
         int n = (int)(r / (Ho * Wo));
         int rem = (int)(r - (int64_t)n * Ho * Wo);
         int oh = rem / Wo, ow = rem - oh * Wo;
-        const int hs = oh * 2 - 1, ws = ow * 2 - 1;
-        float4 best = make_float4(-INFINITY, -INFINITY, -INFINITY, -INFINITY);
-        int bi[4] = {-1, -1, -1, -1};
-#pragma unroll
-        for (int kh = 0; kh < 3; ++kh) {
-            int ih = hs + kh;
-            if (ih < 0 || ih >= H) continue;
-#pragma unroll
-            for (int kw = 0; kw < 3; ++kw) {
-                int iw = ws + kw;
-                if (iw < 0 || iw >= W) continue;
-                float4 v = ld4(x + ((size_t)(n * H + ih) * W + iw) * C + c);
-                const int tap = kh * 3 + kw;
-                if (bi[0] < 0 || v.x > best.x || v.x != v.x) { best.x = v.x; bi[0] = tap; }
-                if (bi[1] < 0 || v.y > best.y || v.y != v.y) { best.y = v.y; bi[1] = tap; }
-                if (bi[2] < 0 || v.z > best.z || v.z != v.z) { best.z = v.z; bi[2] = tap; }
-                if (bi[3] < 0 || v.w > best.w || v.w != v.w) { best.w = v.w; bi[3] = tap; }
-            }
-        }
+        float4 best;
+        uchar4 u;
+        pool_scan4(x, n, oh, ow, H, W, C, c, tap, best, u);
         st4x(y, (int64_t)r * C + c, yps, best);
-        uchar4 u = make_uchar4((unsigned char)bi[0], (unsigned char)bi[1], (unsigned char)bi[2],
-                               (unsigned char)bi[3]);
         *reinterpret_cast<uchar4*>(idx + (size_t)r * C + c) = u;
     }
+}
+
+__global__ __launch_bounds__(256) void k_maxpool_fwd(const float* __restrict__ x, int N, int H, int W, int C4,
+                                                     void* __restrict__ y, int64_t yps, uint8_t* __restrict__ idx, int Ho,
+                                                     int Wo, int CQ, int RL) {
+    RowThread rt = row_thread(C4, CQ, RL);
+    if (!rt.active) return;
+    maxpool_fwd_rows(rt, x, N, H, W, C4, PoolTapPlain(), y, yps, idx, Ho, Wo);
+}
+
+__global__ __launch_bounds__(256) void k_bn_relu_maxpool_fwd(const float* __restrict__ x, int N, int H, int W, int C4,
+                                                             const float* __restrict__ scale, const float* __restrict__ shift,
+                                                             const float* __restrict__ mean, void* __restrict__ y, int64_t yps,
+                                                             uint8_t* __restrict__ idx, int Ho, int Wo, int CQ, int RL) {
+    RowThread rt = row_thread(C4, CQ, RL);
+    if (!rt.active) return;
+    const int c = rt.c4 * 4;
+    const PoolTapBnRelu tap = {ld4(mean + c), ld4(scale + c), ld4(shift + c)};
+    maxpool_fwd_rows(rt, x, N, H, W, C4, tap, y, yps, idx, Ho, Wo);
 }
 
 __global__ __launch_bounds__(256) void k_maxpool_bwd(const float* __restrict__ dy,
@@ -47,31 +59,8 @@
     if (!rt.active) return;
     const int C = C4 * 4, c = rt.c4 * 4;
     const int64_t Mi = (int64_t)N * H * W;
-    for (int64_t r = rt.row0; r < Mi; r += rt.rstep) {
-        int n = (int)(r / (H * W));
-        int rem = (int)(r - (int64_t)n * H * W);
-        int ih = rem / W, iw = rem - ih * W;
-        float4 g = make_float4(0, 0, 0, 0);
-        const int oh_lo = ih >> 1, oh_hi = (ih + 1) >> 1;
-        const int ow_lo = iw >> 1, ow_hi = (iw + 1) >> 1;
-        for (int oh = oh_lo; oh <= oh_hi; ++oh) {
-            if (oh >= Ho) continue;
-            const int kh = ih - (oh * 2 - 1);
-            for (int ow = ow_lo; ow <= ow_hi; ++ow) {
-                if (ow >= Wo) continue;
-                const int kw = iw - (ow * 2 - 1);
-                const unsigned char tap = (unsigned char)(kh * 3 + kw);
-                size_t o = ((size_t)(n * Ho + oh) * Wo + ow) * C + c;
-                uchar4 u = *reinterpret_cast<const uchar4*>(idx + o);
-                float4 d = ld4(dy + o);
-                if (u.x == tap) g.x += d.x;
-                if (u.y == tap) g.y += d.y;
-                if (u.z == tap) g.z += d.z;
-                if (u.w == tap) g.w += d.w;
-            }
-        }
-        st4(dx + (size_t)r * C + c, g);
-    }
+    const PoolGradRows rows = {dy, idx, H, W, Ho, Wo, C};
+    for (int64_t r = rt.row0; r < Mi; r += rt.rstep) st4(dx + (size_t)r * C + c, rows(r, c));
 }
 
 __global__ __launch_bounds__(256) void k_gap_fwd(const void* __restrict__ x, int64_t xps, int HW, int C4, int ldx,
@@ -200,9 +189,28 @@
     return check_launch("maxpool_fwd");
 }
 
+extern "C" int iswm_bn_relu_maxpool3x3s2_fwd_pl(const float* y, int N, int H, int W, int C, const float* scale,
+                                                const float* shift, const float* mean, void* out, int64_t out_ps,
+                                                uint8_t* idx, int Ho, int Wo, iswm_stream_t stream) {
+    ISWM_REQUIRE(y && scale && shift && mean && out && idx && C > 0 && C % 4 == 0 && N > 0 && H > 0 && W > 0,
+                 "bn_relu_maxpool_fwd: bad argument");
+    ISWM_REQUIRE(out_ps == 0 || out_ps == -1 || (out_ps >= (int64_t)N * Ho * Wo * C && out_ps % 4 == 0),
+                 "bn_relu_maxpool_fwd: bad plane stride");
+    ISWM_REQUIRE(Ho == (H + 2 - 3) / 2 + 1 && Wo == (W + 2 - 3) / 2 + 1, "bn_relu_maxpool_fwd: bad output size");
+    ISWM_REQUIRE(aligned16(y) && aligned16(scale) && aligned16(shift) && aligned16(mean) &&
+                     (out_ps == 0 ? aligned16(out) : (reinterpret_cast<uintptr_t>(out) & 7) == 0) &&
+                     (reinterpret_cast<uintptr_t>(idx) & 3) == 0,
+                 "bn_relu_maxpool_fwd: misaligned tensor");
+    RowPlan p = plan_rows((int64_t)N * Ho * Wo, C);
+    hipLaunchKernelGGL(k_bn_relu_maxpool_fwd, dim3(p.rowblocks, p.colblocks), dim3(256), 0, (hipStream_t)stream, y, N, H, W,
+                       p.C4, scale, shift, mean, out, out_ps, idx, Ho, Wo, p.CQ, p.RL);
+    return check_launch("bn_relu_maxpool_fwd");
+}
+
 extern "C" int iswm_maxpool3x3s2_bwd(const float* dy, const uint8_t* idx, int N, int H, int W, int C, int Ho,
                                      int Wo, float* dx, iswm_stream_t stream) {
     ISWM_REQUIRE(dy && idx && dx && C % 4 == 0 && N > 0, "maxpool_bwd: bad argument");
+    ISWM_REQUIRE((int64_t)N * H * W <= INT32_MAX, "maxpool_bwd: map of 2^31 pixels or more");
     RowPlan p = plan_rows((int64_t)N * H * W, C);
     hipLaunchKernelGGL(k_maxpool_bwd, dim3(p.rowblocks, p.colblocks), dim3(256), 0, (hipStream_t)stream, dy, idx,
                        N, H, W, p.C4, Ho, Wo, dx, p.CQ, p.RL);
diff --git a/iswm_amd/csrc/pool_window.h b/iswm_amd/csrc/pool_window.h
--- /dev/null
+++ b/iswm_amd/csrc/pool_window.h
@@ -0,0 +1,71 @@
+#pragma once
+#include "rowmap.h"
+
+namespace iswm {
+
+template <typename Tap>
+__device__ __forceinline__ void pool_scan4(const float* __restrict__ x, int n, int oh, int ow, int H, int W, int C, int c,
+                                           const Tap& tap_value, float4& best, uchar4& arg) {
+    const int hs = oh * 2 - 1, ws = ow * 2 - 1;
+    best = make_float4(-INFINITY, -INFINITY, -INFINITY, -INFINITY);
+    int bi[4] = {-1, -1, -1, -1};
+#pragma unroll
+    for (int kh = 0; kh < 3; ++kh) {
+        int ih = hs + kh;
+        if (ih < 0 || ih >= H) continue;
+#pragma unroll
+        for (int kw = 0; kw < 3; ++kw) {
+            int iw = ws + kw;
+            if (iw < 0 || iw >= W) continue;
+            const float4 v = tap_value(ld4(x + ((size_t)(n * H + ih) * W + iw) * C + c));
+            const int tap = kh * 3 + kw;
+            if (bi[0] < 0 || v.x > best.x || v.x != v.x) { best.x = v.x; bi[0] = tap; }
+            if (bi[1] < 0 || v.y > best.y || v.y != v.y) { best.y = v.y; bi[1] = tap; }
+            if (bi[2] < 0 || v.z > best.z || v.z != v.z) { best.z = v.z; bi[2] = tap; }
+            if (bi[3] < 0 || v.w > best.w || v.w != v.w) { best.w = v.w; bi[3] = tap; }
+        }
+    }
+    arg = make_uchar4((unsigned char)bi[0], (unsigned char)bi[1], (unsigned char)bi[2], (unsigned char)bi[3]);
+}
+
+__device__ __forceinline__ float4 pool_gather4(const float* __restrict__ dy, const uint8_t* __restrict__ idx, int n, int ih,
+                                               int iw, int Ho, int Wo, int C, int c) {
+    const int oh0 = ih >> 1, oh1 = (ih + 1) >> 1, ow0 = iw >> 1, ow1 = (iw + 1) >> 1;
+    const bool vh1 = oh1 != oh0 && oh1 < Ho, vw1 = ow1 != ow0 && ow1 < Wo;
+    const int ohs[2] = {oh0, vh1 ? oh1 : oh0}, ows[2] = {ow0, vw1 ? ow1 : ow0};
+    const bool vhs[2] = {true, vh1}, vws[2] = {true, vw1};
+    uchar4 u[4];
+    float4 d[4];
+#pragma unroll
+    for (int k = 0; k < 4; ++k) {
+        const size_t o = ((size_t)(n * Ho + ohs[k >> 1]) * Wo + ows[k & 1]) * C + c;
+        u[k] = *reinterpret_cast<const uchar4*>(idx + o);
+        d[k] = ld4(dy + o);
+    }
+    float4 g = make_float4(0, 0, 0, 0);
+#pragma unroll
+    for (int k = 0; k < 4; ++k) {
+        const int kh = ih - (ohs[k >> 1] * 2 - 1), kw = iw - (ows[k & 1] * 2 - 1);
+        const unsigned char tap = (unsigned char)(kh * 3 + kw);
+        const bool on = vhs[k >> 1] && vws[k & 1];
+        if (on && u[k].x == tap) g.x += d[k].x;
+        if (on && u[k].y == tap) g.y += d[k].y;
+        if (on && u[k].z == tap) g.z += d[k].z;
+        if (on && u[k].w == tap) g.w += d[k].w;
+    }
+    return g;
+}
+
+struct PoolGradRows {
+    const float* dy;
+    const uint8_t* idx;
+    int H, W, Ho, Wo, C;
+    __device__ __forceinline__ float4 operator()(int64_t r, int c) const {
+        const unsigned ru = (unsigned)r, hw = (unsigned)(H * W);
+        const unsigned nu = ru / hw, rem = ru - nu * hw, ihu = rem / (unsigned)W;
+        const int n = (int)nu, ih = (int)ihu, iw = (int)(rem - ihu * (unsigned)W);
+        return pool_gather4(dy, idx, n, ih, iw, Ho, Wo, C, c);
+    }
+};
+
+}
diff --git a/iswm_amd/csrc/rowmap.h b/iswm_amd/csrc/rowmap.h
--- a/iswm_amd/csrc/rowmap.h
+++ b/iswm_amd/csrc/rowmap.h
@@ -54,4 +54,10 @@
 __device__ __forceinline__ float4 ld4(const float* p) { return *reinterpret_cast<const float4*>(p); }
 __device__ __forceinline__ void st4(float* p, float4 v) { *reinterpret_cast<float4*>(p) = v; }
 
+__device__ __forceinline__ float bn_fwd1(float v, float mu, float sc, float sh) { return __fmaf_rn(__fsub_rn(v, mu), sc, sh); }
+__device__ __forceinline__ float4 bn_fwd4(const float4 v, const float4 mu, const float4 sc, const float4 sh) {
+    return make_float4(bn_fwd1(v.x, mu.x, sc.x, sh.x), bn_fwd1(v.y, mu.y, sc.y, sh.y), bn_fwd1(v.z, mu.z, sc.z, sh.z),
+                       bn_fwd1(v.w, mu.w, sc.w, sh.w));
 }
+
+}
diff --git a/iswm_amd/network/_hip.py b/iswm_amd/network/_hip.py
--- a/iswm_amd/network/_hip.py
+++ b/iswm_amd/network/_hip.py
@@ -354,7 +354,10 @@
         want_planes = ops.planes_on() and y.shape[3] % 64 == 0
     else:
         want_planes = out_fmt == "planes" and ops.planes_on() and y.shape[3] % 64 == 0
-    o = ops.bn_apply(y, coef, relu, residual, out, planes=want_planes)
+    if isinstance(residual, tuple):
+        o = ops.bn_apply_res_bn(y, coef, residual[0], residual[1], relu, out, planes=want_planes)
+    else:
+        o = ops.bn_apply(y, coef, relu, residual, out, planes=want_planes)
     if MASK_RECORDER is not None and relu:
         of = ops.as_f32(o)
         MASK_RECORDER[bn] = (of > 0) & (of < 6) if relu == 6 and relu is not True else (of > 0)
@@ -364,6 +367,64 @@
     if save:
         ctx = dict(x=x, y=y, out=o, coef=coef, g=g, relu=relu, training=training, res=residual is not None, sep=sep, dw=dw)
     return o, ctx
+
+
+_DS_FUSE = True
+_STEM_FUSE = True
+
+
+def ds_fusable(conv, bn):
+    return (_DS_FUSE and CALIB_RECORDER is None and ops.nplanes() != 1 and type(conv) is Conv2d and conv.bias is None and
+            bn.momentum is not None and bn.track_running_stats and bn.affine)
+
+
+def cba_fwd_deferred(conv, bn, x, save):
+    g = conv.geometry(x)
+    training = bn.training
+    y, partials, tiles = ops.conv2d_fwd(x, conv.weight_for(0), g, want_stats=training)
+    coef = _bn_coef(bn, y, partials, tiles, training)
+    ctx = None
+    if save:
+        ctx = dict(x=x, y=y, out=None, coef=coef, g=g, relu=False, training=training, res=False, sep=None, dw=False)
+    return (y, coef), ctx
+
+
+def stem_fusable(conv, bn, pool):
+    return (_STEM_FUSE and CALIB_RECORDER is None and type(conv) is Conv2d and conv.bias is None and conv.cout_p % 4 == 0 and
+            isinstance(pool, nn.MaxPool2d) and (pool.kernel_size, pool.stride, pool.padding) == (3, 2, 1) and
+            pool.dilation == 1 and not pool.ceil_mode and
+            bn.momentum is not None and bn.track_running_stats and bn.affine)
+
+
+def relu_pattern_of(y, coef):
+    z = (y - coef[2]).double() * coef[0].double() + coef[1].double()
+    return z > 2.0 ** -150
+
+
+def cba_pool_fwd(conv, bn, pool, x, save):
+    g = conv.geometry(x)
+    training = bn.training
+    y, partials, tiles = ops.conv2d_fwd(x, conv.weight_for(0), g, want_stats=training)
+    coef = _bn_coef(bn, y, partials, tiles, training)
+    pooled, idx = ops.bn_relu_maxpool_fwd(y, coef, planes=ops.planes_on() and y.shape[3] % 64 == 0)
+    if POOL_RECORDER is not None:
+        POOL_RECORDER[pool] = idx
+    if MASK_RECORDER is not None:
+        MASK_RECORDER[bn] = relu_pattern_of(y, coef)
+    ctx = dict(x=x, y=y, coef=coef, g=g, training=training, idx=idx) if save else None
+    return pooled, ctx
+
+
+def cba_pool_bwd(conv, bn, ctx, dpool, sink, need_dx=True):
+    x, y, g = ctx["x"], ctx["y"], ctx["g"]
+    dgamma, dbeta = _bn_grad_targets(bn, sink)
+    dyp = ops.planes_conv_ok(conv.cin_p, conv.cout_p, 1) and (need_dx or ops.is_planes(x))
+    dy = ops.bn_backward_maxpool(ops.as_f32(dpool), ctx["idx"], y, ctx["coef"], bn.weight, ctx["training"], dgamma, dbeta, dyp)
+    _bn_grads_done(bn, sink)
+    conv.write_wgrad(x, dy, g, sink)
+    if not need_dx:
+        return None
+    return ops.conv2d_dgrad(dy, conv.weight_for(1), g, tuple(x.shape))
 
 
 _BN3_FUSE = True
diff --git a/iswm_amd/network/backbone/resnet.py b/iswm_amd/network/backbone/resnet.py
--- a/iswm_amd/network/backbone/resnet.py
+++ b/iswm_amd/network/backbone/resnet.py
@@ -42,7 +42,9 @@
         o1, c1 = _hip.cba_fwd(self.conv1, self.bn1, True, x, save)
         o2, c2 = _hip.cba_fwd(self.conv2, self.bn2, True, o1, save)
         identity, cd = x, None
-        if self.downsample is not None:
+        if self.downsample is not None and _hip.ds_fusable(self.downsample[0], self.downsample[1]):
+            identity, cd = _hip.cba_fwd_deferred(self.downsample[0], self.downsample[1], x, save)
+        elif self.downsample is not None:
             identity, cd = _hip.cba_fwd(self.downsample[0], self.downsample[1], False, x, save)
         out, c3 = _hip.cba_fwd(self.conv3, self.bn3, True, o2, save, residual=identity)
         self._saved = (c1, c2, c3, cd) if save else None
diff --git a/iswm_amd/network/utils.py b/iswm_amd/network/utils.py
--- a/iswm_amd/network/utils.py
+++ b/iswm_amd/network/utils.py
@@ -138,11 +138,16 @@
     def fwd(self, x, save):
         out = OrderedDict()
         stem_ctx = None
+        pooled = (list(self._modules)[:4] == ["conv1", "bn1", "relu", "maxpool"] and
+                  not {"conv1", "bn1", "relu"} & set(self.return_layers) and
+                  _hip.stem_fusable(self["conv1"], self["bn1"], self["maxpool"]))
         for name, module in self.named_children():
-            if name == "conv1":
+            if name == "conv1" and pooled:
+                x, stem_ctx = _hip.cba_pool_fwd(self["conv1"], self["bn1"], self["maxpool"], x, save)
+            elif name == "conv1":
                 fmt = "f32" if "maxpool" in self._modules else None
                 x, stem_ctx = _hip.cba_fwd(self["conv1"], self["bn1"], True, x, save, out_fmt=fmt)
-            elif name in ("bn1", "relu"):
+            elif name in ("bn1", "relu") or (name == "maxpool" and pooled):
                 pass
             else:
                 x = module.fwd(x, save)
@@ -157,13 +162,16 @@
         tap = {inv[k]: g for k, g in dfeats.items() if g is not None}
         dy = None
         order = list(reversed(names))
+        pooled = self._saved is not None and "idx" in self._saved
         for k, name in enumerate(order):
             if name in tap:
                 g = tap.pop(name)
                 dy = g if dy is None else ops.add_inplace(dy, g)
-            if name in ("relu", "bn1"):
+            if name in ("relu", "bn1") or (name == "maxpool" and pooled):
                 continue
-            if name == "conv1":
+            if name == "conv1" and pooled:
+                dy = _hip.cba_pool_bwd(self["conv1"], self["bn1"], self._saved, dy, sink, need_dx=need_dx)
+            elif name == "conv1":
                 dy, _ = _hip.cba_bwd(self["conv1"], self["bn1"], self._saved, dy, sink, need_dx=need_dx)
             else:
                 below = order[k + 1] if k + 1 < len(order) else None
diff --git a/iswm_amd/ops.py b/iswm_amd/ops.py
--- a/iswm_amd/ops.py
+++ b/iswm_amd/ops.py
@@ -679,6 +679,44 @@
     return out
 
 
+def bn_apply_res_bn(y, coef, yr, coef_r, relu, out=None, planes=False):
+    m, c, ldy = rows(y)
+    mr, cr, ldyr = rows(yr)
+    assert (mr, cr) == (m, c) and nplanes() != 1
+    if out is None:
+        out = new_planes(*y.shape, y.device) if planes else torch.empty(y.shape, dtype=torch.float32, device=y.device)
+    po, mo, co, ldo, pso = xrows(out)
+    assert (mo, co) == (m, c)
+    call("iswm_bn_apply_res_bn_pl", _p(y), m, c, ldy, _p(coef[0]), _p(coef[1]), _p(coef[2]), _p(yr), ldyr, _p(coef_r[0]),
+         _p(coef_r[1]), _p(coef_r[2]), _relu_code(relu), _p(po), ldo, pso, _stream())
+    return out
+
+
+def bn_relu_maxpool_fwd(y, coef, planes=False):
+    n, h, w, c, ld = geom(y)
+    assert ld == c
+    ho, wo = (h + 2 - 3) // 2 + 1, (w + 2 - 3) // 2 + 1
+    out = new_planes(n, ho, wo, c, y.device) if planes else new_act(n, ho, wo, c, y.device)
+    po, _, _, _, _, _, ps = xgeom(out)
+    idx = torch.empty((n, ho, wo, c), dtype=torch.uint8, device=y.device)
+    call("iswm_bn_relu_maxpool3x3s2_fwd_pl", _p(y), n, h, w, c, _p(coef[0]), _p(coef[1]), _p(coef[2]), _p(po), ps, _p(idx), ho,
+         wo, _stream())
+    return out, idx
+
+
+def bn_backward_maxpool(dpool, idx, y, coef, gamma, training, dgamma, dbeta, dy_planes=False):
+    n, h, w, c, ldy = geom(y)
+    _, ho, wo, cp, ldp = geom(dpool)
+    assert ldp == c and cp == c and tuple(idx.shape) == (n, ho, wo, c) and idx.is_contiguous()
+    need = _lib.load().iswm_bn_bwd_workspace(n * h * w, c)
+    ws = torch.empty((need // 8,), dtype=torch.float64, device=y.device)
+    dy = new_planes(*y.shape, y.device) if dy_planes else torch.empty(y.shape, dtype=torch.float32, device=y.device)
+    pdy, _, _, lddy, psdy = xrows(dy)
+    call("iswm_bn_backward_maxpool", _p(dpool), _p(idx), n, h, w, ho, wo, _p(y), ldy, c, _p(coef[2]), _p(coef[3]), _p(gamma),
+         _p(coef[0]), _p(coef[1]), int(bool(training)), _p(dgamma), _p(dbeta), _p(pdy), lddy, psdy, _p(ws), need, _stream())
+    return dy
+
+
 def bn_backward(dout, out, y, coef, gamma, relu, training, dgamma, dbeta, want_dres=False, dy=None, dy_planes=False,
                 stats=None):
     m, c, ldy = rows(y)
```

Measured after the change: 280.2 images/sec (median of 6 runs). No clear change (+0.9%).
